# trevor-vincent/disco4est

Hardware: AMD Instinct MI355X
Metric: GDoF/s for matrix-free 3D DG stiffness apply (Ax), p=7 (higher is better)
Workload: dtype f64; 1 GPU; 3D Poisson stiffness apply on a single-tree brick, uniform level=4 (4096 elements/GPU), p=7, deg_quad=deg+0, Gauss-Legendre; general path (per-node symmetric metric streamed, affine values); dofs_per_gpu=2097152, elements_per_gpu=4096

## Files before the change

disco4est_amd/csrc/d4est_hip_direct.hip:

```cpp
#include <algorithm>
#include <type_traits>

#include "d4est_hip_direct.h"
#include "d4est_hip_internal.h"
#include "d4est_hip_tables.h"
#include "d4est_hip_wave.h"

namespace d4est_hip {

#ifndef D4EST_HIP_DIRECT_IMM_ROWS
#define D4EST_HIP_DIRECT_IMM_ROWS 1
#endif
#if D4EST_HIP_DIRECT_IMM_ROWS
#define D4EST_DIRECT_ROWS contract_rows_eo_imm
#else
#define D4EST_DIRECT_ROWS contract_rows_eo
#endif
template <int NI, int NO, bool EO, bool ANTI>
__device__ __forceinline__ void prod(const double* __restrict__ tab, const double* x, double* y) {
  if constexpr (EO) {
    constexpr int HC = (NI + 1) / 2;
    double xe[HC], xo[HC], ab[NO];
    eo_pre<NI>(x, xe, xo);
    D4EST_DIRECT_ROWS<HC, NO, false>(tab, ANTI ? xo : xe, ANTI ? xe : xo, ab);
    eo_post<NO>(ab, y);
  } else {
    contract_n<NI, NO>(tab, x, y);
  }
}

template <int NI, int NO, bool EO>
__device__ __forceinline__ void prod_pair(const double* __restrict__ tabS, const double* __restrict__ tabA, const double* x, double* yS,
                                          double* yA) {
  if constexpr (EO) {
    constexpr int HC = (NI + 1) / 2;
    double xe[HC], xo[HC], abS[NO], abA[NO];
    eo_pre<NI>(x, xe, xo);
    D4EST_DIRECT_ROWS<HC, NO, false>(tabS, xe, xo, abS);
    D4EST_DIRECT_ROWS<HC, NO, false>(tabA, xo, xe, abA);
    eo_post<NO>(abS, yS);
    eo_post<NO>(abA, yA);
  } else {
    contract_n<NI, NO>(tabS, x, yS);
    contract_n<NI, NO>(tabA, x, yA);
  }
}

template <int N>
__device__ __forceinline__ double row_dot(const double* __restrict__ drow, const double* x) {
  sdouble_ptr row = launder(drow);
  double s = row[0] * x[0];
#pragma unroll
  for (int i = 1; i < N; ++i) s = fma(row[i], x[i], s);
  return s;
}

constexpr int cmax(int a, int b) { return a > b ? a : b; }

template <int N, int NQ>
struct DirectCfg {
  static_assert(NQ >= N && NQ * NQ <= 64, "one wavefront per element: (deg_quad + 1)^2 <= 64");
  static constexpr int N2 = N * N, N3 = N2 * N, T = NQ * NQ, PN = N | 1;
  static constexpr int RS = N | 1, RQ = NQ | 1;
  static constexpr int GS = NQ * RS, YS = N * RQ;
  static constexpr int QS = T + 8, VS = N2 + 8;
  static constexpr int S_DOUBLES = cmax(cmax(cmax(8 * N * RS, 8 * GS), cmax(8 * QS, 8 * NQ * RQ)), cmax(8 * YS, 6 * VS));
  static constexpr int U_DOUBLES = PN * N2;
  static constexpr int OPSZ = N * NQ;
  static constexpr bool FULL = (N == 8 && NQ == 8);
};

constexpr int kDirectWPB = 4;

#ifndef D4EST_HIP_DIRECT_NT_MASK
#define D4EST_HIP_DIRECT_NT_MASK 7
#endif
#ifndef D4EST_HIP_DIRECT_GEOM_EARLY
#define D4EST_HIP_DIRECT_GEOM_EARLY 1
#endif
#ifndef D4EST_HIP_DIRECT_GEOM_NT_RT
#define D4EST_HIP_DIRECT_GEOM_NT_RT 1
#endif
template <int T, bool NT = false , bool HANG = false >
__device__ __forceinline__ void direct_load_geom(double* gq, int kind, bool on, int k, int sgeom, const double* __restrict__ geom,
                                                 const double* __restrict__ robin_c, bool nt_rt = false) {
#pragma unroll
  for (int c = 0; c < 7; ++c) gq[c] = 0.0;
  if (on && !(HANG && kind == 3)) {
    if (kind == 0 && robin_c) {
      gq[6] = robin_c[sgeom + k];
    } else {
      const double* __restrict__ g = geom + (size_t)7 * sgeom + k;
      if (!NT && D4EST_HIP_DIRECT_GEOM_NT_RT && nt_rt) {
        const double* gn = g;
        asm volatile("" : "+v"(gn));
#pragma unroll
        for (int c = 0; c < 7; ++c) gq[c] = __builtin_nontemporal_load(&gn[c * T]);
      } else {
#pragma unroll
        for (int c = 0; c < 7; ++c) gq[c] = ld_sel<NT>(&g[c * T]);
      }
    }
  }
}

template <int N, int NQ, bool EO, bool FUSE, int VOL = 0 >
__global__ __launch_bounds__(64 * kDirectWPB, 4) void faces_direct_kernel(const double* __restrict__ u, const double* __restrict__ ghost_qtrace,
                                                             double* __restrict__ Au, const DirectSide* __restrict__ sides,
                                                             const DirectGhostOff* __restrict__ ghost_off,
                                                             const double* __restrict__ ops, const double* __restrict__ geom,
                                                             const double* __restrict__ bndry_q, const double* __restrict__ robin_c,
                                                             const double* __restrict__ robin_r, int n_elem, int ns0, int ns_stride,
                                                             int xcd_chunk, DirectFuse cf, DirectVol vol, const int* __restrict__ elem_list) {
  using C = DirectCfg<N, NQ>;
  constexpr int N2 = C::N2, N3 = C::N3, T = C::T, PN = C::PN, RS = C::RS, RQ = C::RQ, GS = C::GS, QS = C::QS, YS = C::YS, VS = C::VS;
  constexpr bool FULL = C::FULL;
  constexpr int L0 = cmax(C::U_DOUBLES, VOL ? WaveCfg<N, NQ>::FS : 0), L1 = cmax(C::S_DOUBLES, VOL ? WaveCfg<N, NQ>::FS : 0);
  __shared__ double s_L[kDirectWPB][L0 + L1];
  const int wv = __builtin_amdgcn_readfirstlane(threadIdx.x >> 6);
  double* s_U = s_L[wv];
  double* s_S = s_L[wv] + L0;
#define tC (ops)
#define tCD (ops + C::OPSZ)
#define tE (ops + 2 * C::OPSZ)
#define tDtE (ops + 3 * C::OPSZ)
#define dr0 (ops + 4 * C::OPSZ)
  const int lane = threadIdx.x & 63;
  const int a = lane % NQ, b = lane / NQ;
  const bool on_q = FULL || lane < T, on_m = FULL || (on_q && a < N && b < N);
  const int v = blockIdx.x;
  const int slot = (xcd_chunk > 0 ? (v & 7) * xcd_chunk + (v >> 3) : v) * kDirectWPB + wv;
  if (slot >= n_elem) return;
  const int e = elem_list ? __builtin_amdgcn_readfirstlane(elem_list[slot]) : slot;
  const int ns = __builtin_amdgcn_readfirstlane(ns_stride >= 0 ? ns0 + e * ns_stride : direct_kargs()->sides[6 * (size_t)e].pad);

  {
    constexpr int UT = (N3 + 63) / 64;
    double uo[UT];
#pragma unroll
    for (int t = 0; t < UT; ++t) uo[t] = (N3 % 64 == 0 || lane + 64 * t < N3) ? u[ns + lane + 64 * t] : 0.0;
#pragma unroll
    for (int t = 0; t < UT; ++t) {
      const int idx = lane + 64 * t;
      const int i = idx % N, j = (idx / N) % N, k = idx / N2;
      if (N3 % 64 == 0 || idx < N3) s_U[i + PN * (j + N * k)] = uo[t];
    }
  }
  wave_lds_fence();
  double own_tr[6], own_nd[6];
  {
    sdouble_ptr r0 = launder(dr0), r1 = launder(dr0 + N);
#pragma unroll
    for (int d = 0; d < 3; ++d) {
      double x[N];
#pragma unroll
      for (int i = 0; i < N; ++i) {
        const int idx = (d == 0) ? i + PN * (a + N * b) : (d == 1 ? a + PN * (i + N * b) : a + PN * (b + N * i));
        x[i] = on_m ? lds_ld(&s_U[idx]) : 0.0;
      }
      own_tr[2 * d] = x[0];
      own_tr[2 * d + 1] = x[N - 1];
      double s0 = r0[0] * x[0], s1 = r1[0] * x[0];
#pragma unroll
      for (int i = 1; i < N; ++i) {
        s0 = fma(r0[i], x[i], s0);
        s1 = fma(r1[i], x[i], s1);
      }
      own_nd[2 * d] = s0;
      own_nd[2 * d + 1] = s1;
    }
  }
  wave_lds_fence();

  double facc[N];
#pragma unroll
  for (int i = 0; i < N; ++i) facc[i] = 0.0;
  int any3 = 0;

  auto dir_body = [&](auto dc) {
    constexpr int d = decltype(dc)::value;
    constexpr int t0 = (d == 0) ? 1 : 0, t1d = (d == 2) ? 1 : 2;
    typedef const DirectSide __attribute__((address_space(4))) * sside_ptr;
    const sside_ptr sd = (sside_ptr)(unsigned long long)(direct_kargs()->sides + 6 * (size_t)e);
    const int kcf[2] = {sd[2 * d].kcf, sd[2 * d + 1].kcf};
    const int sgeom[2] = {sd[2 * d].geom, sd[2 * d + 1].geom};
    if constexpr ((VOL & 16) != 0 && FUSE) any3 |= ((kcf[0] & 3) == 3) | ((kcf[1] & 3) == 3);
    double fld[8] = {own_tr[2 * d], own_tr[2 * d + 1], 0.0, 0.0, own_nd[2 * d], own_nd[2 * d + 1], 0.0, 0.0};
    double yy[2][N];
#pragma unroll
    for (int h = 0; h < 2; ++h) {
#pragma unroll
      for (int i = 0; i < N; ++i) yy[h][i] = 0.0;
      if ((kcf[h] & 3) == 1 && on_m) {
        const double* __restrict__ up = u + sd[2 * d + h].nbr_ns;
        const int dp = kcf[h] >> 6;
        const int st = (dp == 0) ? 1 : (dp == 1 ? N : N2);
        const int o0 = (dp == 0) ? N * a + N2 * b : (dp == 1 ? a + N2 * b : a + N * b);
#pragma unroll
        for (int i = 0; i < N; ++i) yy[h][i] = up[o0 + st * i];
      }
    }
#if D4EST_HIP_DIRECT_GEOM_EARLY == 2
    double gqa[2][7];
#pragma unroll
    for (int h = 0; h < 2; ++h) direct_load_geom<T, (VOL & 8) != 0 && (D4EST_HIP_DIRECT_NT_MASK & 1) != 0, (VOL & 16) != 0>(gqa[h], kcf[h] & 3, on_q, lane, sgeom[h], direct_kargs()->geom, direct_kargs()->robin_c);
#endif
#pragma unroll
    for (int h = 0; h < 2; ++h) {
      if ((kcf[h] & 3) == 1) {
        const int hi = (kcf[h] >> 5) & 1;
        fld[2 + h] = hi ? yy[h][N - 1] : yy[h][0];
        fld[6 + h] = row_dot<N>(dr0 + hi * N, yy[h]);
      }
    }
    wave_lds_fence();
    if (on_m) {
#pragma unroll
      for (int c = 0; c < 8; ++c) s_S[(c * N + b) * RS + a] = fld[c];
    }
    wave_lds_fence();
    const bool row_on = FULL || lane < 8 * N;
    const int rc = lane / N, rb = lane % N;
    double P[NQ], R[NQ];
    {
      double x[N];
#pragma unroll
      for (int i = 0; i < N; ++i) x[i] = row_on ? lds_ld(&s_S[lane * RS + i]) : 0.0;
      prod_pair<N, NQ, EO>(tC, tCD, x, P, R);
    }
// ... 55 lines not shown
        const int k = lane;
#pragma unroll
        for (int c = 0; c < 4; ++c) qm[c] = lds_ld(&s_S[c * QS + k]);
        if (kind == 1) {
          const int kp = reorder_index(code, NQ - 1, a, b);
#pragma unroll
          for (int c = 0; c < 4; ++c) qp[c] = lds_ld(&s_S[(4 + c) * QS + kp]);
        } else if (kind == 2) {
          const double* __restrict__ p = K->ghost_qtrace + K->ghost_off[6 * (size_t)e + 2 * d + h] + reorder_index(code, NQ - 1, a, b);
#pragma unroll
          for (int c = 0; c < 4; ++c) qp[c] = p[c * T];
        } else if ((VOL & 16) != 0 && kind == 3) {
        } else if (robin_c) {
          qp[0] = K->robin_r[sgeom[h] + k];
        } else {
          qp[0] = K->bndry_q[sgeom[h] + k];
        }
#if D4EST_HIP_DIRECT_GEOM_EARLY == 0
        direct_load_geom<T, (VOL & 8) != 0 && (D4EST_HIP_DIRECT_NT_MASK & 1) != 0, (VOL & 16) != 0>(gq, kind, true, k, sgeom[h], geom, robin_c);
#endif
        if constexpr ((VOL & 16) != 0) {
          const int xoff = sd[2 * d + h].nbr_ns;
          if (kind == 2 && xoff >= 0) {
            double* __restrict__ tp = const_cast<double*>((const double*)K->ghost_qtrace) + xoff;
#pragma unroll
            for (int c = 0; c < 4; ++c) tp[c * T + k] = qm[c];
          }
        }
      }
#if D4EST_HIP_DIRECT_GEOM_EARLY != 0
#pragma unroll
      for (int c = 0; c < 7; ++c) gq[c] = gqa[h][c];
#endif
      double t1 = 0.0;
#pragma unroll
      for (int i = 0; i < 3; ++i) t1 += gq[i] * qm[1 + i] + gq[3 + i] * qp[1 + i];
      const double jump = qm[0] - qp[0];
      const double w1 = (kind != 0) ? -0.5 : -1.0;
      At[h][0] = (kind == 0 && robin_c) ? gq[6] * qm[0] - qp[0] : w1 * t1 + gq[6] * jump;
#pragma unroll
      for (int l = 0; l < 3; ++l) At[h][1 + l] = w1 * gq[l] * jump;
    }
    wave_lds_fence();
    if (on_q) {
#pragma unroll
      for (int h = 0; h < 2; ++h)
#pragma unroll
        for (int c = 0; c < 4; ++c) s_S[((4 * h + c) * NQ + b) * RQ + a] = At[h][c];
    }
    wave_lds_fence();
    double Yv[N];
    {
      double row[NQ];
#pragma unroll
      for (int q = 0; q < NQ; ++q) row[q] = col_on ? lds_ld(&s_S[lane * RQ + q]) : 0.0;
      if ((cc & 3) == 1 + t0) prod<NQ, N, EO, true>(tDtE, row, Yv);
      else prod<NQ, N, EO, false>(tE, row, Yv);
    }
    wave_lds_fence();
    if (col_on) {
#pragma unroll
      for (int i = 0; i < N; ++i) s_S[cc * YS + i * RQ + aq] = Yv[i];
    }
    wave_lds_fence();
    const bool v_on = lane < 6 * N;
    const int vh = lane / (3 * N), vg = (lane / N) % 3, va = lane % N;
    double Vv[N];
    {
      double colq[NQ];
      const int f1 = (vg == 0) ? 0 : (vg == 1 ? 1 + t1d : 1 + d);
#pragma unroll
      for (int q = 0; q < NQ; ++q) {
        double t = v_on ? lds_ld(&s_S[(4 * vh + f1) * YS + va * RQ + q]) : 0.0;
        if (v_on && vg == 0) t += lds_ld(&s_S[(4 * vh + 1 + t0) * YS + va * RQ + q]);
        colq[q] = t;
      }
      if (vg == 1) prod<NQ, N, EO, true>(tDtE, colq, Vv);
      else prod<NQ, N, EO, false>(tE, colq, Vv);
    }
    wave_lds_fence();
    if (v_on) {
#pragma unroll
      for (int i = 0; i < N; ++i) s_S[(3 * vh + vg) * VS + i * N + va] = Vv[i];
    }
    wave_lds_fence();
    double acc[N];
    if (on_m) {
      const double val0 = lds_ld(&s_S[0 * VS + b * N + a]) + lds_ld(&s_S[1 * VS + b * N + a]), n0 = lds_ld(&s_S[2 * VS + b * N + a]);
      const double val1 = lds_ld(&s_S[3 * VS + b * N + a]) + lds_ld(&s_S[4 * VS + b * N + a]), n1 = lds_ld(&s_S[5 * VS + b * N + a]);
      sdouble_ptr r0 = launder(dr0), r1 = launder(dr0 + N);
#pragma unroll
      for (int i = 0; i < N; ++i) acc[i] = fma(r0[i], n0, r1[i] * n1);
      acc[0] += val0;
      acc[N - 1] += val1;
      if constexpr (d == 0) {
#pragma unroll
        for (int i = 0; i < N; ++i) s_U[i + PN * (a + N * b)] = acc[i];
      } else if constexpr (d == 1) {
#pragma unroll
        for (int i = 0; i < N; ++i) s_U[a + PN * (i + N * b)] += acc[i];
      } else if constexpr (VOL != 0) {
#pragma unroll
        for (int i = 0; i < N; ++i) facc[i] = lds_ld(&s_U[a + PN * (b + N * i)]) + acc[i];
      } else {
        DirectFuse cfl;
        if constexpr (FUSE) cfl = direct_load_fuse(direct_kargs());
        double* __restrict__ Au_ = direct_kargs()->Au;
        double av[N], rh[FUSE ? N : 1], pp[FUSE ? N : 1], uu[FUSE ? N : 1];
#pragma unroll
        for (int i = 0; i < N; ++i) {
          const size_t o = (size_t)ns + a + N * b + N2 * i;
          av[i] = Au_[o];
          if constexpr (FUSE) { rh[i] = cfl.rhs[o]; pp[i] = cfl.p[o]; uu[i] = u[o]; }
        }
#pragma unroll
        for (int i = 0; i < N; ++i) {
          const size_t o = (size_t)ns + a + N * b + N2 * i;
          const double au = av[i] + (lds_ld(&s_U[a + PN * (b + N * i)]) + acc[i]);
          Au_[o] = au;
          if constexpr (FUSE) {
            const double res = __dadd_rn(rh[i], __dmul_rn(-1.0, au));
            const double ri = __dmul_rn(cfl.alpha, res);
            const double pi = __dadd_rn(__dmul_rn(cfl.beta, pp[i]), ri);
            if (cfl.r) cfl.r[o] = ri;
            cfl.p[o] = pi;
            cfl.u_out[o] = __dadd_rn(uu[i], pi);
          }
        }
      }
    }
    wave_lds_fence();
  };
  dir_body(std::integral_constant<int, 0>{});
  dir_body(std::integral_constant<int, 1>{});
  dir_body(std::integral_constant<int, 2>{});
  if constexpr (VOL != 0) {
    static_assert(VOL == 0 || N == NQ, "fused volume term: N = NQ");
    {
      constexpr int UT = (N3 + 63) / 64;
      double uo[UT];
#pragma unroll
      for (int t = 0; t < UT; ++t) uo[t] = (N3 % 64 == 0 || lane + 64 * t < N3) ? u[ns + lane + 64 * t] : 0.0;
#pragma unroll
      for (int t = 0; t < UT; ++t) {
        const int idx = lane + 64 * t;
        const int i = idx % N, j = (idx / N) % N, k = idx / N2;
        if (N3 % 64 == 0 || idx < N3) s_U[i + PN * (j + N * k)] = uo[t];
      }
    }
    wave_lds_fence();
    {
      const DirectVol vl = direct_load_vol(direct_kargs());
      const int qs = __builtin_amdgcn_readfirstlane(vl.qs_stride >= 0 ? vl.qs0 + e * vl.qs_stride : vl.qs_list[e]);
      stiffness_wave_eo_element<N, NQ, (VOL & 3) == 2, false, (VOL & 4) != 0, (VOL & 8) != 0 && (D4EST_HIP_DIRECT_NT_MASK & 2) != 0>(s_U, s_S, vl.metric, qs, e, on_q, a, b, vl.EBf, vl.EGf, vl.EBb,
                                                                              vl.EGb, vl.affine, vl.wq, vl.cq);
    }
    if (on_m) {
      DirectFuse cfl;
      if constexpr (FUSE) cfl = direct_load_fuse(direct_kargs());
      double* __restrict__ Au_ = direct_kargs()->Au;
      const bool upd = !((VOL & 16) != 0 && any3 != 0);
      double rh[FUSE ? N : 1], pp[FUSE ? N : 1], uu[FUSE ? N : 1];
      if constexpr (FUSE) {
        if (upd) {
#pragma unroll
          for (int i = 0; i < N; ++i) {
            const size_t o = (size_t)ns + a + N * b + N2 * i;
            rh[i] = cfl.rhs[o]; pp[i] = cfl.p[o]; uu[i] = u[o];
          }
        }
      }
#pragma unroll
      for (int i = 0; i < N; ++i) {
        const size_t o = (size_t)ns + a + N * b + N2 * i;
        const double au = s_U[a + PN * (b + N * i)] + facc[i];
        if constexpr (!FUSE && (VOL & 8) != 0 && (D4EST_HIP_DIRECT_NT_MASK & 4) != 0) __builtin_nontemporal_store(au, &Au_[o]);
        else if (!FUSE || !cfl.skip_Au_store || !upd) Au_[o] = au;
        if (FUSE && upd) {
          const double res = __dadd_rn(rh[i], __dmul_rn(-1.0, au));
          const double ri = __dmul_rn(cfl.alpha, res);
          const double pi = __dadd_rn(__dmul_rn(cfl.beta, pp[i]), ri);
          if (cfl.r) cfl.r[o] = ri;
          cfl.p[o] = pi;
          cfl.u_out[o] = __dadd_rn(uu[i], pi);
        }
      }
    }
  }
#undef tC
#undef tCD
#undef tE
#undef tDtE
#undef dr0
}

static DirectHost* host_of(d4est_hip_plan* plan) { return static_cast<DirectHost*>(plan->direct); }

void direct_destroy(d4est_hip_plan* plan) {
  DirectHost* dh = host_of(plan);
  if (!dh) return;
  (void)hipFree(dh->d_sides);
  (void)hipFree(dh->d_ghost_off);
  (void)hipFree(dh->d_ops);
  (void)hipFree(dh->d_u2);
  (void)hipFree(dh->d_bnd_list); (void)hipFree(dh->d_int_list);
  delete dh;
  plan->direct = nullptr;
}

#define D4EST_HIP_DIRECT_PAIRS(X) X(2, 2) X(3, 3) X(4, 4) X(5, 5) X(6, 6) X(7, 7) X(8, 8) X(2, 3) X(3, 4) X(4, 5) X(3, 6) X(4, 6)

static bool direct_pair_built(int N, int NQ) {
#define X(N_, NQ_) if (N == N_ && NQ == NQ_) return true;
  D4EST_HIP_DIRECT_PAIRS(X)
#undef X
  return direct_mw_built(N, NQ);
}

void direct_setup(d4est_hip_plan* plan, int N, int NQ, int ns0, int ns_stride, const double* Cm, const double* CDm, const double* Em) {
  direct_destroy(plan);
  if (!direct_pair_built(N, NQ)) return;
  const int ne = plan->n_elements;
  DirectHost* dh = new DirectHost;
  dh->N = N; dh->NQ = NQ; dh->ns0 = ns0; dh->ns_stride = ns_stride;
  dh->mw = direct_mw_built(N, NQ);
  dh->eo = true;
  std::vector<double> Cv(Cm, Cm + (size_t)NQ * N), CDv(CDm, CDm + (size_t)NQ * N), Ev(Em, Em + (size_t)N * NQ);
  std::vector<double> D = Tables1D::dij(N - 1);
  std::vector<double> DtE = Tables1D::matmul(Tables1D::transpose(D, N, N), Ev, N, N, NQ);
  std::vector<double> ops;
  auto put = [&](const std::vector<double>& M, int R, int Cc, bool anti) {
    std::vector<double> t = dh->eo ? Tables1D::eo_table(M, R, Cc, anti) : Tables1D::transpose(M, R, Cc);
    t.resize((size_t)R * Cc, 0.0);
    ops.insert(ops.end(), t.begin(), t.end());
  };
  put(Cv, NQ, N, false);
  put(CDv, NQ, N, true);
  put(Ev, N, NQ, false);
  put(DtE, N, NQ, true);
  for (int i = 0; i < N; ++i) ops.push_back(D[i]);
  for (int i = 0; i < N; ++i) ops.push_back(D[(size_t)(N - 1) * N + i]);
  ops.resize(ops.size() + 16, 0.0);
  HIP_CHECK(hipMalloc(&dh->d_ops, ops.size() * sizeof(double)));
  HIP_CHECK(hipMemcpy(dh->d_ops, ops.data(), ops.size() * sizeof(double), hipMemcpyHostToDevice));
  std::vector<DirectSide> sd(6 * (size_t)ne);
  std::vector<DirectGhostOff> goff(6 * (size_t)ne, 0);
  for (int e = 0; e < ne; ++e)
    for (int f = 0; f < 6; ++f) {
      const size_t s = 6 * (size_t)e + f;
      DirectSide d{};
      const int nbr = plan->side_nbr[s];
      const int kind = (nbr == -1) ? 0 : (nbr >= 0 ? 1 : 2);
      const int fp = (kind == 0) ? 0 : plan->side_nbr_face[s];
      d.kcf = kind | ((plan->side_reorder[s] & 7) << 2) | (fp << 5);
      d.nbr_ns = (kind == 1) ? plan->nodal_stride[nbr] : 0;
      d.geom = plan->side_mortar_stride[s];
      goff[s] = (kind == 2) ? plan->ghost_trace_offset[s] : 0;
      sd[s] = d;
    }
  HIP_CHECK(hipMalloc(&dh->d_sides, std::max<size_t>(sd.size(), 1) * sizeof(DirectSide)));
  if (!sd.empty()) HIP_CHECK(hipMemcpy(dh->d_sides, sd.data(), sd.size() * sizeof(DirectSide), hipMemcpyHostToDevice));
  HIP_CHECK(hipMalloc(&dh->d_ghost_off, std::max<size_t>(goff.size(), 1) * sizeof(DirectGhostOff)));
  if (!goff.empty()) HIP_CHECK(hipMemcpy(dh->d_ghost_off, goff.data(), goff.size() * sizeof(DirectGhostOff), hipMemcpyHostToDevice));
  std::vector<int> bnd, inn;
  for (int e = 0; e < ne; ++e) {
    bool g = false;
    for (int f = 0; f < 6; ++f) g = g || plan->side_nbr[6 * (size_t)e + f] <= -2;
    (g ? bnd : inn).push_back(e);
  }
  if (!bnd.empty()) {
    dh->n_bnd = (int)bnd.size(); dh->n_int = (int)inn.size();
    HIP_CHECK(hipMalloc(&dh->d_bnd_list, bnd.size() * sizeof(int)));
    HIP_CHECK(hipMemcpy(dh->d_bnd_list, bnd.data(), bnd.size() * sizeof(int), hipMemcpyHostToDevice));
    HIP_CHECK(hipMalloc(&dh->d_int_list, std::max<size_t>(inn.size(), 1) * sizeof(int)));
    if (!inn.empty()) HIP_CHECK(hipMemcpy(dh->d_int_list, inn.data(), inn.size() * sizeof(int), hipMemcpyHostToDevice));
  }
  plan->direct = dh;
}

void direct_ghost_split(d4est_hip_plan* plan, const int** bnd_list, int* n_bnd, const int** int_list, int* n_int) {
  DirectHost* dh = host_of(plan);
  if (!dh) D4EST_HIP_ABORT("direct_ghost_split: the plan has no direct face kernel");
  *bnd_list = dh->d_bnd_list; *n_bnd = dh->n_bnd; *int_list = dh->d_int_list; *n_int = dh->n_int;
}

constexpr int kDirectMinElements = 768;

bool direct_active(const d4est_hip_plan* plan) {
  const int t = plan->tuning[D4EST_HIP_TUNE_FACE_DIRECT];
  const DirectHost* dh = static_cast<const DirectHost*>(plan->direct);
  return dh != nullptr && t != 0 && plan->tuning[D4EST_HIP_TUNE_FLUX_FAST] != 0 &&
         (t > 0 || dh->mw || plan->n_elements >= kDirectMinElements);
}

void direct_set_element_list(d4est_hip_plan* plan, const int* list_dev, int n_list) {
  DirectHost* dh = host_of(plan);
  if (!dh) D4EST_HIP_ABORT("direct_set_element_list: the plan has no direct face kernel");
  dh->d_list = list_dev;
  dh->n_list = list_dev ? n_list : 0;
}

bool direct_has_element_list(const d4est_hip_plan* plan) {
  const DirectHost* dh = static_cast<const DirectHost*>(plan->direct);
  return dh && dh->d_list != nullptr;
}

double* direct_second_vector(d4est_hip_plan* plan) {
  DirectHost* dh = host_of(plan);
  if (!dh->d_u2) HIP_CHECK(hipMalloc(&dh->d_u2, std::max<size_t>((size_t)plan->local_nodes, 1) * sizeof(double)));
  return dh->d_u2;
}

bool direct_fused_ok(const d4est_hip_plan* plan) {
  const DirectHost* dh = static_cast<const DirectHost*>(plan->direct);
  static const bool dbg = std::getenv("D4EST_HIP_DEBUG_FUSED") != nullptr;
  auto no = [&](const char* why) {
    if (dbg) std::fprintf(stderr, "[d4est_hip] whole-operator kernel not used: %s\n", why);
    return false;
  };
  if (!direct_active(plan) || !dh) return no("no direct face kernel on this plan");
  const int t = plan->tuning[D4EST_HIP_TUNE_FACE_DIRECT];
  if (!(t < 0 || t == 2)) return no("tuning key 11");
  if (dh->N != dh->NQ) return no("deg != deg_quad");
  if (!plan->has_geometry) return no("no geometry yet");
  if (plan->buckets.size() != 1) return no("more than one (deg, deg_quad) bucket");
  const Bucket& bk = plan->buckets[0];
  if (bk.N != dh->N || bk.NQ != dh->NQ || !bk.d_EBf) return no("bucket tables");
  if (bk.ns_stride >= 0 && (bk.ns0 != dh->ns0 || bk.ns_stride != dh->ns_stride)) return no("nodal offsets");
  if (bk.n_elem != plan->n_elements) return no("bucket size");
  if (dh->order_ok < 0) {
    int ok = 1;
    for (int i = 0; i < plan->n_elements && ok; ++i) ok = (plan->elem_ids[i] == i);
    dh->order_ok = ok;
  }
  if (!dh->order_ok) return no("bucket order");
  if (dh->mw) {
    if (plan->tuning[D4EST_HIP_TUNE_STIFFNESS_EO] == 0) return no("even-odd contractions switched off");
    return true;
  }
  const int tw = plan->tuning[D4EST_HIP_TUNE_STIFFNESS_WAVE];
  if (!(tw < 0 || tw == 11)) return no("tuning key 1");
  return true;
}

static void launch_direct_core(d4est_hip_plan* plan, DirectHost* dh, const Bucket& bk, bool hybrid, const int* d_qs_by_elem, const double* u,
                               const double* ghost_trace, double* Au, const DirectFuse* cf, const double* robin_c, const double* robin_r,
                               int vol_term) {
  if (!plan->has_face_geometry) D4EST_HIP_ABORT("apply flux: plan_set_mortar_geometry was not called");
  const int n = dh->d_list ? dh->n_list : plan->n_elements;
  if (n == 0) return;
  if (plan->ghost_trace_doubles > 0 && !ghost_trace) D4EST_HIP_ABORT("apply flux: plan has ghost sides but no ghost trace buffer was given");
  static const bool no_remap = std::getenv("D4EST_HIP_NO_XCD_REMAP") != nullptr;
  const int wpb = dh->mw ? 1 : kDirectWPB;
  const int n_wg = (n + wpb - 1) / wpb;
  const int chunk = (n % (8 * wpb) == 0 && !no_remap) ? n_wg / 8 : 0;
  DirectVol vol;
  int vmode = 0;
  if (vol_term) {
    if (!hybrid && !direct_fused_ok(plan)) D4EST_HIP_ABORT("direct face kernel: the fused volume term was requested on a plan that cannot take it");
    vol.metric = plan->d_metric;
    vol.EBf = bk.d_EBf; vol.EGf = bk.d_EGf; vol.EBb = bk.d_EBb; vol.EGb = bk.d_EGb;
    vol.EDq = bk.d_EDq; vol.EDqT = bk.d_EDqT;
    vol.stream = plan->stream_mode;
    {
      static const int geom_nt = [] { const char* e = std::getenv("D4EST_HIP_GEOM_NT"); return e ? std::atoi(e) : 1; }();
      if (!dh->mw && !vol.stream && (geom_nt == 2 || (geom_nt == 1 && hybrid))) vol.stream |= 2;
    }
    if (hybrid && dh->hy_qs_stride > 0) { vol.qs0 = dh->hy_qs0; vol.qs_stride = dh->hy_qs_stride; vol.qs_list = nullptr; }
    else if (hybrid) { vol.qs0 = 0; vol.qs_stride = -1; vol.qs_list = d_qs_by_elem; }
    else { vol.qs0 = bk.qs0; vol.qs_stride = bk.ns_stride >= 0 ? bk.qs_stride : -1; vol.qs_list = plan->d_qs_list + bk.elem_offset; }
    const bool aff = !hybrid && bk.affine && plan->tuning[D4EST_HIP_TUNE_AFFINE] != 0 && plan->d_metric_affine;
    if (aff) { vol.affine = plan->d_metric_affine; vol.wq = bk.d_w; }
    vmode = aff ? 2 : 1;
    if (vol_term == 2) {
      if (!plan->d_lhs_coeff) D4EST_HIP_ABORT("direct face kernel: the zeroth-order term was requested but no coefficient is set");
      vol.cq = ensure_lhs_wjc(plan);
      vmode |= 4;
    }
    const char* sm = (!aff && vol_term != 2 && (vol.stream & 1)) ? ",stream" : "";
    if (dh->mw) std::snprintf(plan->last_kernel, sizeof(plan->last_kernel), "d4est_hip::operator_mw_kernel<%d,vol%s%s> (stiffness_wave_kernel body + faces)", dh->N, aff ? ",affine" : "", sm);
    else std::snprintf(plan->last_kernel, sizeof(plan->last_kernel), "d4est_hip::faces_direct_kernel<%d,%d,vol%s%s> (faces + stiffness_wave_eo body)", dh->N, dh->NQ, aff ? ",affine" : "", sm);
  }
  if (dh->mw) {
    launch_direct_mw(plan, dh, u, ghost_trace, Au, cf, robin_c, robin_r, vmode, vol, n, chunk);
    return;
  }
  const DirectFuse cfv = cf ? *cf : DirectFuse{};
  bool done = false;
  if (vmode == 1 && (vol.stream & 1)) vmode = 9;
  if (dh->hang) {
    if (!(vmode == 1 || vmode == 9)) D4EST_HIP_ABORT("direct face kernel: the hanging-aware form exists for the plain whole operator only (vmode %d)", vmode);
    vmode |= 16;
  }
#define D4EST_HIP_DIRECT_GO(N_, NQ_, FUSE_, VOL_)                                                                             \
  hipLaunchKernelGGL((faces_direct_kernel<N_, NQ_, true, FUSE_, VOL_>), dim3(n_wg), dim3(64 * kDirectWPB), 0,     \
                     plan->stream, u, ghost_trace, Au, dh->d_sides, dh->d_ghost_off, dh->d_ops, plan->d_face_geom, plan->d_bndry,            \
                     robin_c, robin_r, n, dh->ns0, dh->ns_stride, chunk, cfv, vol, dh->d_list)
#define X(N_, NQ_)                                                                 \
  if (!done && dh->N == N_ && dh->NQ == NQ_) {                                     \
    if constexpr (N_ == NQ_) {                                                     \
      if (vmode == 1) { if (cf) D4EST_HIP_DIRECT_GO(N_, NQ_, true, 1); else D4EST_HIP_DIRECT_GO(N_, NQ_, false, 1); done = true; } \
      if (vmode == 9) { if (cf) D4EST_HIP_DIRECT_GO(N_, NQ_, true, 9); else D4EST_HIP_DIRECT_GO(N_, NQ_, false, 9); done = true; } \
      if (vmode == 17) { if (cf) D4EST_HIP_DIRECT_GO(N_, NQ_, true, 17); else D4EST_HIP_DIRECT_GO(N_, NQ_, false, 17); done = true; } \
      if (vmode == 25) { if (cf) D4EST_HIP_DIRECT_GO(N_, NQ_, true, 25); else D4EST_HIP_DIRECT_GO(N_, NQ_, false, 25); done = true; } \
      if (vmode == 2) { if (cf) D4EST_HIP_DIRECT_GO(N_, NQ_, true, 2); else D4EST_HIP_DIRECT_GO(N_, NQ_, false, 2); done = true; } \
      if (vmode == 5) { if (cf) D4EST_HIP_DIRECT_GO(N_, NQ_, true, 5); else D4EST_HIP_DIRECT_GO(N_, NQ_, false, 5); done = true; } \
      if (vmode == 6) { if (cf) D4EST_HIP_DIRECT_GO(N_, NQ_, true, 6); else D4EST_HIP_DIRECT_GO(N_, NQ_, false, 6); done = true; } \
    }                                                                              \
    if (!done) { if (cf) D4EST_HIP_DIRECT_GO(N_, NQ_, true, 0); else D4EST_HIP_DIRECT_GO(N_, NQ_, false, 0); done = true; }        \
  }
  D4EST_HIP_DIRECT_PAIRS(X)
#undef X
#undef D4EST_HIP_DIRECT_GO
  if (!done) D4EST_HIP_ABORT("direct face kernel: no instance for N = %d, NQ = %d", dh->N, dh->NQ);
  static bool occ_done = false;
  if (!occ_done && std::getenv("D4EST_HIP_DEBUG_OCC")) {
    occ_done = true;
    int nb = -1, nv = -1;
    hipFuncAttributes at{}, av{};
    (void)hipOccupancyMaxActiveBlocksPerMultiprocessor(&nb, reinterpret_cast<const void*>(faces_direct_kernel<8, 8, true, false, 0>), 64 * kDirectWPB, 0);
    (void)hipFuncGetAttributes(&at, reinterpret_cast<const void*>(faces_direct_kernel<8, 8, true, false, 0>));
    (void)hipOccupancyMaxActiveBlocksPerMultiprocessor(&nv, reinterpret_cast<const void*>(faces_direct_kernel<8, 8, true, false, 1>), 64 * kDirectWPB, 0);
    (void)hipFuncGetAttributes(&av, reinterpret_cast<const void*>(faces_direct_kernel<8, 8, true, false, 1>));
    std::fprintf(stderr, "[d4est_hip] occupancy: faces_direct<8,8> %d workgroups of %d waves per CU (regs %d, lds %zu, scratch %zu); with the volume term %d (regs %d, lds %zu, scratch %zu)\n",
                 nb, kDirectWPB, at.numRegs, at.sharedSizeBytes, at.localSizeBytes, nv, av.numRegs, av.sharedSizeBytes, av.localSizeBytes);
  }
  HIP_CHECK(hipGetLastError());
}

void launch_direct_faces(d4est_hip_plan* plan, const double* u, const double* ghost_trace, double* Au, const DirectFuse* cf,
                         const double* robin_c, const double* robin_r, int vol_term) {
  DirectHost* dh = host_of(plan);
  if (!dh) D4EST_HIP_ABORT("direct face kernel: the plan has no direct tables");
  launch_direct_core(plan, dh, plan->buckets[0], false, nullptr, u, ghost_trace, Au, cf, robin_c, robin_r, vol_term);
}

struct HybridHost {
  std::vector<DirectHost*> dh;
  std::vector<int*> d_clean;
  std::vector<int> n_clean;
  DirectSide* d_sides = nullptr;
  DirectGhostOff* d_ghost_off = nullptr;
  int* d_qs_by_elem = nullptr;
  int *d_dirty = nullptr, *d_ring = nullptr;
  int n_dirty = 0, n_ring = 0, n_clean_total = 0;
  std::vector<int> h_dirty, h_ring;
  int *d_ns_dirty = nullptr, *d_qs_dirty = nullptr;
  std::vector<int> dirty_off, dirty_cnt;
  char path[96] = "";
  double* d_u2 = nullptr;
  bool hang = false;
  std::vector<hipStream_t> side;
  std::vector<hipEvent_t> done;
  hipEvent_t fork = nullptr;
};
static HybridHost* hybrid_of(const d4est_hip_plan* plan) { return static_cast<HybridHost*>(plan->hybrid); }

void hybrid_destroy(d4est_hip_plan* plan) {
  HybridHost* hh = hybrid_of(plan);
  if (!hh) return;
  for (DirectHost* d : hh->dh)
    if (d) { (void)hipFree(d->d_ops); delete d; }
  for (int* p : hh->d_clean) (void)hipFree(p);
  for (hipStream_t st : hh->side) (void)hipStreamDestroy(st);
  for (hipEvent_t ev : hh->done) (void)hipEventDestroy(ev);
  if (hh->fork) (void)hipEventDestroy(hh->fork);
  (void)hipFree(hh->d_sides); (void)hipFree(hh->d_ghost_off); (void)hipFree(hh->d_qs_by_elem); (void)hipFree(hh->d_dirty); (void)hipFree(hh->d_ring);
  (void)hipFree(hh->d_ns_dirty); (void)hipFree(hh->d_qs_dirty); (void)hipFree(hh->d_u2);
  delete hh;
  plan->hybrid = nullptr;
}

bool hybrid_pair_built(int N, int NQ) { return N == NQ && direct_pair_built(N, NQ); }

template <typename T>
static T* hy_upload(const std::vector<T>& v) {
  T* d = nullptr;
  HIP_CHECK(hipMalloc(&d, std::max<size_t>(v.size(), 1) * sizeof(T)));
  if (!v.empty()) HIP_CHECK(hipMemcpy(d, v.data(), v.size() * sizeof(T), hipMemcpyHostToDevice));
  return d;
}

void hybrid_setup(d4est_hip_plan* plan, const std::vector<char>& clean, const std::vector<const double*>& C, const std::vector<const double*>& CD,
                  const std::vector<const double*>& E, const std::vector<HybridSideOverride>* ov, const char* form) {
  hybrid_destroy(plan);
  const int ne = plan->n_elements;
  HybridHost* hh = new HybridHost;
  const size_t nb = plan->buckets.size();
  hh->dh.assign(nb, nullptr); hh->d_clean.assign(nb, nullptr); hh->n_clean.assign(nb, 0);
  hh->dirty_off.assign(nb, 0); hh->dirty_cnt.assign(nb, 0);
  std::vector<DirectSide> sd(6 * (size_t)ne);
  std::vector<DirectGhostOff> goff(6 * (size_t)ne, 0);
  for (int e = 0; e < ne; ++e)
    for (int f = 0; f < 6; ++f) {
      const size_t s = 6 * (size_t)e + f;
      DirectSide d{};
      const int nbr = plan->side_nbr[s];
      const int kind = (nbr == -1) ? 0 : (nbr >= 0 ? 1 : 2);
      const int fp = (kind == 0) ? 0 : plan->side_nbr_face[s];
      d.kcf = kind | ((plan->side_reorder[s] & 7) << 2) | (fp << 5);
      d.nbr_ns = (kind == 1) ? plan->nodal_stride[nbr] : 0;
      d.geom = plan->side_mortar_stride[s];
      d.pad = (f == 0) ? plan->nodal_stride[e] : 0;
      if (ov && clean[e] && (*ov)[s].kind >= 0) {
        const HybridSideOverride& o = (*ov)[s];
        d.kcf = o.kind | ((plan->side_reorder[s] & 7) << 2);
        if (o.kind == 2) { d.nbr_ns = o.export_off; d.geom = o.geom; goff[s] = o.goff; }
        hh->hang = true;
      }
      sd[s] = d;
    }
  hh->d_sides = hy_upload(sd);
  hh->d_ghost_off = hy_upload(goff);
  hh->d_qs_by_elem = hy_upload(plan->quad_stride);
  std::vector<int> dirty, ns_dirty, qs_dirty;
  for (size_t b = 0; b < nb; ++b) {
    const Bucket& bk = plan->buckets[b];
    std::vector<int> cl;
    hh->dirty_off[b] = (int)ns_dirty.size();
    for (int i = 0; i < bk.n_elem; ++i) {
      const int e = plan->elem_ids[bk.elem_offset + i];
      if (clean[e]) cl.push_back(e);
      else { ns_dirty.push_back(plan->nodal_stride[e]); qs_dirty.push_back(plan->quad_stride[e]); }
    }
    hh->dirty_cnt[b] = (int)ns_dirty.size() - hh->dirty_off[b];
    if (cl.empty()) continue;
    std::sort(cl.begin(), cl.end());
    DirectHost* dh = new DirectHost;
    const int N = bk.N, NQ = bk.NQ;
    dh->N = N; dh->NQ = NQ; dh->ns0 = 0; dh->ns_stride = -1;
    dh->mw = direct_mw_built(N, NQ);
    dh->eo = true;
    dh->hang = hh->hang;
    std::vector<double> Cv(C[b], C[b] + (size_t)NQ * N), CDv(CD[b], CD[b] + (size_t)NQ * N), Ev(E[b], E[b] + (size_t)N * NQ);
// ... 159 lines not shown
```

disco4est_amd/csrc/d4est_hip_internal.h:

```cpp
#pragma once
#include <hip/hip_runtime.h>

#include <cstdio>
#include <cstdlib>
#include <vector>

#include "../../include/d4est_hip.h"

#define D4EST_HIP_ABORT(...)                                   \
  do {                                                         \
    std::fprintf(stderr, "[D4EST_HIP_ABORT] ");                \
    std::fprintf(stderr, __VA_ARGS__);                         \
    std::fprintf(stderr, " (%s:%d)\n", __FILE__, __LINE__);    \
    std::abort();                                              \
  } while (0)

#define HIP_CHECK(expr)                                                              \
  do {                                                                               \
    hipError_t _e = (expr);                                                          \
    if (_e != hipSuccess) D4EST_HIP_ABORT("%s failed: %s", #expr, hipGetErrorString(_e)); \
  } while (0)

namespace d4est_hip {

struct Bucket {
  int deg = 0, deg_quad = 0;
  int N = 0, NQ = 0;
  int n_elem = 0;
  int elem_offset = 0;
  double* d_B = nullptr;
  double* d_G = nullptr;
  double* d_D = nullptr;
  double* d_w = nullptr;
  double* d_BT = nullptr;
  double* d_GT = nullptr;
  double* d_DT = nullptr;
  int ns0 = 0, ns_stride = -1, qs0 = 0, qs_stride = -1;
  bool affine = false;
  double* d_EBf = nullptr;
  double* d_EGf = nullptr;
  double* d_EBb = nullptr;
  double* d_EGb = nullptr;
  double* d_EDq = nullptr;
  double* d_EDqT = nullptr;
  double* d_M = nullptr;
  double* d_MT = nullptr;
  double* d_Minv = nullptr;
  double* d_MinvT = nullptr;
  double* d_Binv = nullptr;
  double* d_BinvT = nullptr;
  double* d_wGL = nullptr;
};

}

struct d4est_hip_plan {
  int n_elements = 0;
  int local_nodes = 0;
  int local_nodes_quad = 0;
  int quad_type = 0;
  hipStream_t stream = nullptr;
  int n_cus = 0;
  char last_kernel[128] = "";

  std::vector<int> deg, deg_quad, nodal_stride, quad_stride;
  std::vector<d4est_hip::Bucket> buckets;

  std::vector<int> elem_ids;
  int* d_elem_ids = nullptr;
  int* d_ns_list = nullptr;
  int* d_qs_list = nullptr;

  bool has_geometry = false;
  double* d_J = nullptr;
  int* d_face_stride = nullptr;
  int face_nodes = 0;
  double* d_metric = nullptr;
  double* d_metric_affine = nullptr;
  int* d_nonaffine = nullptr;

  bool has_faces = false, has_face_geometry = false;
  int n_ghost = 0;
  std::vector<int> ghost_deg, ghost_deg_quad;
  std::vector<int> side_nbr, side_nbr_face, side_reorder, side_mortar_stride, side_bndry_stride;
  std::vector<int> side_hang, side_sub, side_nbr4, side_orientation;
  int total_mortar_nodes = 0, total_bndry_nodes = 0;
  long long local_trace_doubles = 0, ghost_trace_doubles = 0;
  int* d_side_desc = nullptr;
  void* d_elem_desc = nullptr;
  std::vector<long long> rec_qoff, rec_goff;
  std::vector<int> rec_len, side_first_rec;
  std::vector<long long> trace_offset, ghost_trace_offset;
  double* d_face_ops = nullptr;
  double* d_face_geom = nullptr;
  double* d_bndry = nullptr;
  double* d_trace = nullptr;
  double sipg_prefactor = 10.0;
  int sipg_penalty_fcn = 0;
  int max_face_lds_doubles = 0;
  bool face_fast = false;
  void* direct = nullptr;
  void* hybrid = nullptr;

  double *d_work_p = nullptr, *d_work_d = nullptr, *d_work_r = nullptr, *d_reduce = nullptr, *d_ghost_trace = nullptr;
  const double* d_lhs_coeff = nullptr;
  double* d_lhs_c = nullptr;
  double* d_lhs_wjc = nullptr;
  bool lhs_wjc_valid = false;
  double* d_work_m = nullptr;
  const double* d_lhs_blocks = nullptr;
  long long* d_lhs_block_off = nullptr;
  void* lhs_chain = nullptr;
  hipStream_t side_stream = nullptr;
  hipEvent_t ev_fork = nullptr, ev_join = nullptr;
  hipGraphExec_t cheby_graph = nullptr;
  struct { const void *u, *rhs, *Au, *r; int iter, flag; double lmin, lmax; hipStream_t stream; } cheby_graph_key = {};
  d4est_hip_exchange_fn exchange_fn = nullptr;
  d4est_hip_allreduce_fn allreduce_fn = nullptr;
  void* comm_ctx = nullptr;

  unsigned long long op_generation = 0;
  bool quad_aliased = false;
  int stream_mode = 0;
  bool bc_inhomogeneous = false;

  int tuning[D4EST_HIP_TUNE_COUNT] = {-1, -1, -1, -1, -1, -1, -1, -1, -1, -1, -1, -1, -1, -1, -1, -1};

  void* krylov = nullptr;

  double* d_scratch = nullptr;
  size_t scratch_doubles = 0;

  bool est_requested = false;
  int est_fcn[3] = {-1, -1, -1};
  double est_prefactor = 0.0;
  void* est = nullptr;

  double* h_stage = nullptr;
  double* d_host[4] = {nullptr, nullptr, nullptr, nullptr};
};

namespace d4est_hip {
struct TreeMapParams;
struct CellDesc;
void launch_analytic_geometry(d4est_hip_plan* plan, const TreeMapParams& P, const CellDesc* d_cells, double root_len);
void faces_set_geometry_analytic(d4est_hip_plan* plan, const TreeMapParams& P, const std::vector<CellDesc>& elem,
                                 const std::vector<CellDesc>& ghost, double root_len);

void launch_metric_precombine(d4est_hip_plan* plan, const double* d_J, const double* d_rst);
void launch_stiffness(d4est_hip_plan* plan, const double* u, double* Au);
void launch_stiffness_view(d4est_hip_plan* plan, const double* u, double* Au, int* ns_list_view, int* qs_list_view, const int* view_offset,
                           const int* view_count);
void launch_mass_like(d4est_hip_plan* plan, int mode, const double* in, double* out, const double* coeff = nullptr, int which = 0);
void launch_brick_geometry(d4est_hip_plan* plan, const int* d_elem_dq, double root_len, const double* extents);
void launch_numerical_geometry(d4est_hip_plan* plan, const double* d_xyz);
void faces_set_geometry_brick(d4est_hip_plan* plan, const int* d_elem_dq, double root_len, const double* extents);
void launch_slicer_lift(d4est_hip_plan* plan, const double* in, double* out, int face, int lift);
void launch_dij(d4est_hip_plan* plan, const double* in, double* out, int dir, int transpose);
void launch_dudr(d4est_hip_plan* plan, const double* u, double* d0, double* d1, double* d2);

void faces_setup(d4est_hip_plan* plan);
void faces_set_geometry(d4est_hip_plan* plan, const double* sj, const double* n, const double* drst_m, const double* drst_p,
                        const double* hm, const double* hp, int on_device);
int reorient_face_order(int f_m, int f_p, int o, int i);
int face_reorder_code(int f_m, int f_p, int o);
void faces_set_dirichlet(d4est_hip_plan* plan, const double* g_lobatto, int on_device);
void faces_set_robin(d4est_hip_plan* plan, const double* coeff_quad, const double* rhs_quad, int on_device);
void launch_traces(d4est_hip_plan* plan, const double* u, double* trace, bool ghost, const int* elist = nullptr, int n_list = 0, int parts = 3 );
struct ChebyFuse {
  const double* rhs = nullptr;
  double* p = nullptr;
  double* u = nullptr;
  double* u_out = nullptr;
  int skip_Au_store = 0;
  double* r = nullptr;
  double alpha = 0.0, beta = 0.0;
};
bool flux_can_fuse_update(d4est_hip_plan* plan);

struct DirectFuse {
  const double* rhs = nullptr;
  double* p = nullptr;
  double* u_out = nullptr;
  double* r = nullptr;
  double alpha = 0.0, beta = 0.0;
  int skip_Au_store = 0;
  int pad = 0;
};
void direct_setup(d4est_hip_plan* plan, int N, int NQ, int ns0, int ns_stride, const double* C, const double* CD, const double* E);
void direct_destroy(d4est_hip_plan* plan);
bool direct_active(const d4est_hip_plan* plan);
double* direct_second_vector(d4est_hip_plan* plan);
void direct_set_element_list(d4est_hip_plan* plan, const int* list_dev, int n_list);
bool direct_has_element_list(const d4est_hip_plan* plan);
bool direct_fused_ok(const d4est_hip_plan* plan);
void direct_ghost_split(d4est_hip_plan* plan, const int** bnd_list, int* n_bnd, const int** int_list, int* n_int);
void launch_direct_faces(d4est_hip_plan* plan, const double* u, const double* ghost_trace, double* Au, const DirectFuse* cf,
                         const double* robin_c, const double* robin_r, int vol_term);
void launch_flux_direct(d4est_hip_plan* plan, const double* u, const double* ghost_trace, double* Au, const DirectFuse* cf = nullptr,
                        int vol_term = 0);
void launch_flux(d4est_hip_plan* plan, const double* trace, const double* ghost_trace, double* Au, const ChebyFuse* cf = nullptr,
                 const int* elist = nullptr, int n_list = 0, int parts = 3);
bool hybrid_pair_built(int N, int NQ);
struct HybridSideOverride { int kind; long long goff; int export_off; int geom; };
void hybrid_setup(d4est_hip_plan* plan, const std::vector<char>& clean, const std::vector<const double*>& C, const std::vector<const double*>& CD,
                  const std::vector<const double*>& E, const std::vector<HybridSideOverride>* ov = nullptr, const char* form = "hanging-aware");
bool hybrid_hanging(const d4est_hip_plan* plan);
void hybrid_host_lists(const d4est_hip_plan* plan, const std::vector<int>** dirty, const std::vector<int>** ring);
void hybrid_destroy(d4est_hip_plan* plan);
bool hybrid_active(const d4est_hip_plan* plan);
const char* hybrid_path(const d4est_hip_plan* plan);
void hybrid_lists(const d4est_hip_plan* plan, const int** dirty, int* n_dirty, const int** ring, int* n_ring);
void launch_hybrid_clean(d4est_hip_plan* plan, const double* u, const double* ghost_trace, double* Au, const double* robin_c, const double* robin_r,
                         int phase, const DirectFuse* cf = nullptr);
bool hybrid_can_fuse_update(const d4est_hip_plan* plan);
double* hybrid_second_vector(d4est_hip_plan* plan);
void launch_flux_units(d4est_hip_plan* plan, const double* trace, const double* ghost_trace, double* Au, const ChebyFuse* cf);
bool faces_have_units(d4est_hip_plan* plan);
bool faces_hp(d4est_hip_plan* plan);
bool faces_hp_split(d4est_hip_plan* plan);
void launch_hybrid_dirty_stiffness(d4est_hip_plan* plan, const double* u, double* Au);
void launch_flux_hybrid_clean(d4est_hip_plan* plan, const double* u, const double* ghost_trace, double* Au, int phase, const DirectFuse* cf = nullptr);
void faces_destroy(d4est_hip_plan* plan);
struct EstMortar {
  int elem;
  int kind;
  int code;
  int NQ;
  int gidx;
  int S, off, off_p, Ttot;
  int deg_m, deg_p;
  int N;
  int offC, ops_hp;
  int bstride;
  int u_shift;
  double fm, fp;
  long long qoff, nbr_qoff;
};
void faces_estimator_mortars(d4est_hip_plan* plan, std::vector<EstMortar>& out, std::vector<int>& elem_first, const double** face_ops,
                             const double** hp_ops);
void launch_traces_all(d4est_hip_plan* plan, const double* u, double* trace);
void launch_boundary_gather(d4est_hip_plan* plan, const double* vol, double* out);
void estimator_setup(d4est_hip_plan* plan, const double* sj, const double* n, const double* drst_m, const double* drst_p, const double* hm,
                     const double* hp);
void estimator_destroy(d4est_hip_plan* plan);
void estimator_compute(d4est_hip_plan* plan, const double* u, const double* ghost_trace, const double* residual, const double* diam,
                       const double* g_lobatto, double* eta2, double* terms);

void apply_operator(d4est_hip_plan* plan, const double* u, double* Au, const ChebyFuse* cf = nullptr, bool lhs_term = true);
void launch_residual(d4est_hip_plan* plan, int n, const double* rhs, const double* Au, double* r);
void launch_residual_inplace(d4est_hip_plan* plan, int n, const double* rhs, double* r);
void launch_residual_inplace_sub(d4est_hip_plan* plan, int n, const double* a, double* r);
void ensure_solver_workspace(d4est_hip_plan* plan);
void add_lhs_mass_term(d4est_hip_plan* plan, const double* u, double* Au);
void add_lhs_blocks_term(d4est_hip_plan* plan, const double* u, double* Au);
void add_lhs_chain_term(d4est_hip_plan* plan, const double* u, double* Au);
void lhs_chain_destroy(d4est_hip_plan* plan);
inline bool lhs_extra_term(const d4est_hip_plan* plan) { return plan->d_lhs_blocks != nullptr || plan->lhs_chain != nullptr; }
const double* ensure_lhs_wjc(d4est_hip_plan* plan);
void launch_copy_blocks(hipStream_t stream, int n_blocks, const double* src, const long long* src_off, double* dst,
                        const long long* dst_off, const int* len);
void launch_dot(d4est_hip_plan* plan, int n, const double* x, const double* y, double* out_dev);
void launch_cheby_update(d4est_hip_plan* plan, int n, const double* rhs, const double* Au, double alpha, double beta, double* r,
                         double* p, double* u);
void cheby_iterate(d4est_hip_plan* plan, double* u, const double* rhs, double* Au, double* r, int iter, double lmin, double lmax,
                   int compute_residual_at_end);
double cg_eigs(d4est_hip_plan* plan, double* u, const double* rhs, double* Au, int imax, int use_new, double* hist_out);

int cg_solve(d4est_hip_plan* plan, double* u, const double* rhs, double* Au, int imax, double atol, double rtol, double* hist_out);
int fcg_solve(d4est_hip_plan* plan, double* u, const double* rhs, double* Au, int imax, double atol, double rtol, d4est_hip_pc_fn pc,
              void* pc_ctx, double* hist_out);
void krylov_destroy(d4est_hip_plan* plan);


}
```

disco4est_amd/csrc/d4est_hip_volume.hip:

```cpp
#include <algorithm>
#include <mutex>
#include <unordered_map>
#include <cstring>

#include "d4est_hip_internal.h"
#include "d4est_hip_maps.h"
#include "d4est_hip_tables.h"
#include "d4est_hip_wave.h"
#include "d4est_hip_mwave.h"

namespace d4est_hip {

template <int N, int NQ>
struct VolCfg {
  static_assert(NQ >= N, "quadrature degree below polynomial degree is served by the generic path");
  static constexpr int PL = NQ * NQ;
  static constexpr int EPB = (PL <= 64) ? (64 / PL) : 1;
  static constexpr int THREADS = (PL <= 64) ? 64 : ((PL + 63) / 64) * 64;
  static constexpr int PN = N | 1;
  static constexpr int PQ = NQ | 1;
  static constexpr int FS = NQ * NQ * PQ;
  static constexpr int LDS_PER_ELEM = 3 * FS;
  static constexpr size_t LDS_BYTES = (size_t)EPB * LDS_PER_ELEM * sizeof(double);
};
// ... 301 lines not shown
      for (int j = 0; j < N; ++j) x[j] = lds_ld(&R1[j + PN * (a + NQ * b)]);
      contract_n_part<N, NQ, HQ>(BopT, q0, x, t_bb);
      contract_n_part<N, NQ, HQ>(GopT, q0, x, t_gb);
#pragma unroll
      for (int j = 0; j < N; ++j) x[j] = lds_ld(&R2[j + PN * (a + NQ * b)]);
      contract_n_part<N, NQ, HQ>(BopT, q0, x, t_bg);
    }
    __syncthreads();
    if (on2) {
#pragma unroll
      for (int jq = 0; jq < HQ; ++jq) {
        R0[b + PN * (a + NQ * (q0 + jq))] = t_bg[jq];
        R1[b + PN * (a + NQ * (q0 + jq))] = t_gb[jq];
        R2[b + PN * (a + NQ * (q0 + jq))] = t_bb[jq];
      }
    }
  }
  __syncthreads();

  double fr[HQ], fs[HQ], ft[HQ];
  if (active) {
    double x[N];
#pragma unroll
    for (int k = 0; k < N; ++k) x[k] = lds_ld(&R0[k + PN * (a + NQ * b)]);
    contract_n_part<N, NQ, HQ>(BopT, q0, x, fr);
#pragma unroll
    for (int k = 0; k < N; ++k) x[k] = lds_ld(&R1[k + PN * (a + NQ * b)]);
    contract_n_part<N, NQ, HQ>(BopT, q0, x, fs);
#pragma unroll
    for (int k = 0; k < N; ++k) x[k] = lds_ld(&R2[k + PN * (a + NQ * b)]);
    contract_n_part<N, NQ, HQ>(GopT, q0, x, ft);
#pragma unroll
    for (int kq = 0; kq < HQ; ++kq) {
      const double r = fr[kq], s = fs[kq], t = ft[kq];
      fr[kq] = mreg[0][kq] * r + mreg[1][kq] * s + mreg[2][kq] * t;
      fs[kq] = mreg[1][kq] * r + mreg[3][kq] * s + mreg[4][kq] * t;
      ft[kq] = mreg[2][kq] * r + mreg[4][kq] * s + mreg[5][kq] * t;
    }
  }
  __syncthreads();
  if (active) {
#pragma unroll
    for (int kq = 0; kq < HQ; ++kq) {
      R0[q0 + kq + PQ * (a + NQ * b)] = fr[kq];
      R1[q0 + kq + PQ * (a + NQ * b)] = fs[kq];
      R2[q0 + kq + PQ * (a + NQ * b)] = ft[kq];
    }
  }
  __syncthreads();
  {
    double x[NQ], ca[HN], cb[HN], cc[HN];
    if (active) {
#pragma unroll
      for (int kq = 0; kq < NQ; ++kq) x[kq] = lds_ld(&R0[kq + PQ * (a + NQ * b)]);
      contract_t_part<NQ, N, HN, false>(Bop, n0, x, ca);
#pragma unroll
      for (int kq = 0; kq < NQ; ++kq) x[kq] = lds_ld(&R1[kq + PQ * (a + NQ * b)]);
      contract_t_part<NQ, N, HN, false>(Bop, n0, x, cb);
#pragma unroll
      for (int kq = 0; kq < NQ; ++kq) x[kq] = lds_ld(&R2[kq + PQ * (a + NQ * b)]);
      contract_t_part<NQ, N, HN, false>(Gop, n0, x, cc);
    }
    __syncthreads();
    if (active) {
#pragma unroll
      for (int k = 0; k < HN; ++k) {
        R0[b + PQ * (a + NQ * (n0 + k))] = ca[k];
        R1[b + PQ * (a + NQ * (n0 + k))] = cb[k];
        R2[b + PQ * (a + NQ * (n0 + k))] = cc[k];
      }
    }
  }
  __syncthreads();
  {
    double x[NQ], ar[HN], bs[HN];
    const bool on6 = active && b < N;
    if (on6) {
#pragma unroll
      for (int jq = 0; jq < NQ; ++jq) x[jq] = lds_ld(&R0[jq + PQ * (a + NQ * b)]);
      contract_t_part<NQ, N, HN, false>(Bop, n0, x, ar);
#pragma unroll
      for (int jq = 0; jq < NQ; ++jq) x[jq] = lds_ld(&R1[jq + PQ * (a + NQ * b)]);
      contract_t_part<NQ, N, HN, false>(Gop, n0, x, bs);
#pragma unroll
      for (int jq = 0; jq < NQ; ++jq) x[jq] = lds_ld(&R2[jq + PQ * (a + NQ * b)]);
      contract_t_part<NQ, N, HN, true>(Bop, n0, x, bs);
    }
    __syncthreads();
    if (on6) {
#pragma unroll
      for (int j = 0; j < HN; ++j) {
        R0[a + PQ * (n0 + j + N * b)] = ar[j];
        R1[a + PQ * (n0 + j + N * b)] = bs[j];
      }
    }
  }
  __syncthreads();
  if (active && a < N && b < N) {
    double x[NQ], o[HN];
#pragma unroll
    for (int iq = 0; iq < NQ; ++iq) x[iq] = lds_ld(&R0[iq + PQ * (a + N * b)]);
    contract_t_part<NQ, N, HN, false>(Gop, n0, x, o);
#pragma unroll
    for (int iq = 0; iq < NQ; ++iq) x[iq] = lds_ld(&R1[iq + PQ * (a + N * b)]);
    contract_t_part<NQ, N, HN, true>(Bop, n0, x, o);
#pragma unroll
    for (int i = 0; i < HN; ++i) R2[n0 + i + PN * (a + N * b)] = o[i];
  }
  __syncthreads();
  if (active) {
#pragma unroll
    for (int idx = te + h * PL; idx < N3; idx += 2 * PL) {
      const int i = idx % N, j = (idx / N) % N, k = idx / (N * N);
      Au[ns + idx] = lds_ld(&R2[i + PN * (j + N * k)]);
    }
  }
}


template <int N, int NQ>
__global__ __launch_bounds__(64, 4) void stiffness_wave2_kernel(
    const double* __restrict__ u, double* __restrict__ Au, const double* __restrict__ metric,
    const int* __restrict__ ns_list, const int* __restrict__ qs_list, int n_bucket, const double* __restrict__ Bop,
    const double* __restrict__ Gop, const double* __restrict__ BopT, const double* __restrict__ GopT, int stagger) {
  if (stagger > 0 && ((blockIdx.x >> 8) & 1)) {
    for (int s_ = 0; s_ < stagger; ++s_) __builtin_amdgcn_s_sleep(16);
  }
  using C = WaveCfg<N, NQ>;
  constexpr int PL = C::PL, PN = C::PN, PQ = C::PQ, FS = C::FS;
  constexpr int N3 = N * N * N, NQ3 = NQ * NQ * NQ;
  extern __shared__ __attribute__((aligned(16))) double smem[];

  const int tid = threadIdx.x;
  const int slot = tid / PL;
  const int te = tid - slot * PL;
  const int a = te % NQ, b = te / NQ;
  const int ei = blockIdx.x * C::EPB + slot;
  const bool active = (slot < C::EPB) && (ei < n_bucket);
  double* R0 = smem + (active ? slot : 0) * C::LDS_PER_ELEM;
  double* R1 = R0 + FS;
  int ns = 0, qs = 0;
  if (active) {
    ns = ns_list[ei];
    qs = qs_list[ei];
    load_element_image<N, PL, PN>(R0, u + ns, te);
  }
  __syncthreads();
  stiffness_wave2_element<N, NQ, true>(R0, R1, metric, qs, active, a, b, Bop, Gop, BopT, GopT);
  if (active) {
    store_element_image<N, PL, PN>(Au + ns, R0, te);
  }
}

template <int N, int NQ, bool AFF = false>
__global__ __launch_bounds__(64, 4) void stiffness_wave_eo_kernel(
    const double* __restrict__ u, double* __restrict__ Au, const double* __restrict__ metric,
    const int* __restrict__ ns_list, const int* __restrict__ qs_list, int n_bucket, const double* __restrict__ EBf,
    const double* __restrict__ EGf, const double* __restrict__ EBb, const double* __restrict__ EGb, int ns0, int ns_stride,
    int qs0, int qs_stride, const double* __restrict__ affine = nullptr, const double* __restrict__ wq = nullptr) {
  using C = WaveCfg<N, NQ>;
  constexpr int PL = C::PL, PN = C::PN, PQ = C::PQ, FS = C::FS;
  constexpr int N3 = N * N * N, NQ3 = NQ * NQ * NQ;
  constexpr int HN = N / 2, HQ = NQ / 2;
  extern __shared__ __attribute__((aligned(16))) double smem[];

  const int tid = threadIdx.x;
  const int slot = tid / PL;
  const int te = tid - slot * PL;
  const int a = te % NQ, b = te / NQ;
  const int ei = blockIdx.x * C::EPB + slot;
  const bool active = (slot < C::EPB) && (ei < n_bucket);
  double* R0 = smem + (active ? slot : 0) * C::LDS_PER_ELEM;
  double* R1 = R0 + FS;
  int ns = 0, qs = 0;
  if (active) {
    if (ns_stride >= 0) {
      ns = ns0 + ei * ns_stride;
      qs = qs0 + ei * qs_stride;
    } else {
      ns = ns_list[ei];
      qs = qs_list[ei];
    }
    if (C::EPB == 1) {
      ns = __builtin_amdgcn_readfirstlane(ns);
      qs = __builtin_amdgcn_readfirstlane(qs);
    }
    load_element_image<N, PL, PN>(R0, u + ns, te);
  }
  __syncthreads();
  stiffness_wave_eo_element<N, NQ, AFF, true>(R0, R1, metric, qs, ei, active, a, b, EBf, EGf, EBb, EGb, affine, wq);
  if (active) {
    store_element_image<N, PL, PN>(Au + ns, R0, te);
  }
}

struct WaveEoMulti {
  static constexpr int MAXB = 7;
  int n = 0;
  int wg_end[MAXB] = {};
  int N[MAXB] = {};
  int n_elem[MAXB] = {};
  int elem_offset[MAXB] = {};
  const double* EBf[MAXB] = {};
  const double* EGf[MAXB] = {};
  const double* EBb[MAXB] = {};
  const double* EGb[MAXB] = {};
  const double* wq[MAXB] = {};
};

template <int N, bool AFF>
__device__ __forceinline__ void wave_eo_multi_body(double* smem, int wg, const double* __restrict__ u, double* __restrict__ Au,
                                                   const double* __restrict__ metric, const int* __restrict__ ns_list,
                                                   const int* __restrict__ qs_list, int n_bucket, const double* __restrict__ EBf,
                                                   const double* __restrict__ EGf, const double* __restrict__ EBb,
                                                   const double* __restrict__ EGb, const double* __restrict__ affine,
                                                   const double* __restrict__ wq) {
  using C = WaveCfg<N, N>;
  constexpr int PL = C::PL, PN = C::PN, FS = C::FS;
  const int tid = threadIdx.x;
  const int slot = tid / PL;
  const int te = tid - slot * PL;
  const int a = te % N, b = te / N;
  const int ei = wg * C::EPB + slot;
  const bool active = (slot < C::EPB) && (ei < n_bucket);
  double* R0 = smem + (active ? slot : 0) * C::LDS_PER_ELEM;
  double* R1 = R0 + FS;
  int ns = 0, qs = 0;
  if (active) {
    ns = ns_list[ei];
    qs = qs_list[ei];
    if (C::EPB == 1) {
      ns = __builtin_amdgcn_readfirstlane(ns);
      qs = __builtin_amdgcn_readfirstlane(qs);
    }
    load_element_image<N, PL, PN>(R0, u + ns, te);
  }
  __syncthreads();
  stiffness_wave_eo_element<N, N, AFF, true>(R0, R1, metric, qs, ei, active, a, b, EBf, EGf, EBb, EGb, affine, wq);
  if (active) {
    store_element_image<N, PL, PN>(Au + ns, R0, te);
  }
}

template <bool AFF>
__global__ __launch_bounds__(64, 4) void stiffness_wave_eo_multi_kernel(const double* __restrict__ u, double* __restrict__ Au,
                                                                        const double* __restrict__ metric,
                                                                        const int* __restrict__ ns_list_all,
                                                                        const int* __restrict__ qs_list_all,
                                                                        const double* __restrict__ affine_all, WaveEoMulti A) {
  extern __shared__ __attribute__((aligned(16))) double smem[];
  const int blk = blockIdx.x;
  int bi = 0;
  while (bi + 1 < A.n && blk >= A.wg_end[bi]) ++bi;
  const int wg = blk - (bi > 0 ? A.wg_end[bi - 1] : 0);
  const int off = A.elem_offset[bi], nb = A.n_elem[bi];
  const double* EBf = A.EBf[bi];
  const double* EGf = A.EGf[bi];
  const double* EBb = A.EBb[bi];
  const double* EGb = A.EGb[bi];
  const double* wq = A.wq[bi];
  const double* aff = AFF ? affine_all + (size_t)6 * off : nullptr;
#define D4EST_CASE(N_)                                                                                                            \
  case N_:                                                                                                                        \
    wave_eo_multi_body<N_, AFF>(smem, wg, u, Au, metric, ns_list_all + off, qs_list_all + off, nb, EBf, EGf, EBb, EGb, aff, wq);   \
    break;
  switch (A.N[bi]) {
    D4EST_CASE(2) D4EST_CASE(3) D4EST_CASE(4) D4EST_CASE(5) D4EST_CASE(6) D4EST_CASE(7) D4EST_CASE(8)
    default: break;
  }
#undef D4EST_CASE
}

template <int N, bool NT>
__device__ __forceinline__ void mw_multi_body(double* smem, int ei, const double* __restrict__ u, double* __restrict__ Au,
                                              const double* __restrict__ metric, const int* __restrict__ ns_list, const int* __restrict__ qs_list,
                                              int n_bucket, const double* __restrict__ EBb, const double* __restrict__ EBf,
                                              const double* __restrict__ EDq, const double* __restrict__ EDqT) {
  using C = WaveCfg<N, N>;
  constexpr int PL = C::PL, PN = C::PN;
  const int te = threadIdx.x;
  const int a = te % N, b = te / N;
  const bool active = (te < PL) && (ei < n_bucket);
  double* R0 = smem;
  double* R1 = R0 + C::FS;
  int ns = 0, qs = 0;
  if (ei < n_bucket) {
    ns = __builtin_amdgcn_readfirstlane(ns_list[ei]);
    qs = __builtin_amdgcn_readfirstlane(qs_list[ei]);
  }
  if (active) load_element_image<N, PL, PN>(R0, u + ns, te);
  stiffness_mw_element_cg<N, false, false, NT>(R0, R1, metric, qs, ei, active, te, a, b, EBb, EBf, EDq, EDqT, nullptr, nullptr);
  if (active) store_element_image<N, PL, PN, NT>(Au + ns, R0, te);
}

template <int THREADS, bool NT>
__global__ __launch_bounds__(THREADS, D4EST_HIP_MW_WAVES) void stiffness_mw_multi_kernel(const double* __restrict__ u, double* __restrict__ Au,
                                                                                        const double* __restrict__ metric,
                                                                                        const int* __restrict__ ns_list_all,
                                                                                        const int* __restrict__ qs_list_all, WaveEoMulti A) {
  extern __shared__ __attribute__((aligned(16))) double smem[];
  const int blk = blockIdx.x;
  int bi = 0;
  while (bi + 1 < A.n && blk >= A.wg_end[bi]) ++bi;
  const int ei = blk - (bi > 0 ? A.wg_end[bi - 1] : 0);
  const int off = A.elem_offset[bi], nb = A.n_elem[bi];
  const double* EBf = A.EBf[bi];
  const double* EDqT = A.EGf[bi];
  const double* EBb = A.EBb[bi];
  const double* EDq = A.EGb[bi];
#define D4EST_CASE(N_)                                                                                                  \
  case N_:                                                                                                              \
    if constexpr (WaveCfg<N_, N_>::THREADS == THREADS)                                                                  \
      mw_multi_body<N_, NT>(smem, ei, u, Au, metric, ns_list_all + off, qs_list_all + off, nb, EBb, EBf, EDq, EDqT);    \
    break;
  switch (A.N[bi]) {
    D4EST_CASE(9) D4EST_CASE(10) D4EST_CASE(11) D4EST_CASE(12) D4EST_CASE(13)
    default: break;
  }
#undef D4EST_CASE
}


template <bool NT>
__global__ __launch_bounds__(128, D4EST_HIP_MW_WAVES) void stiffness_all_multi_kernel(const double* __restrict__ u, double* __restrict__ Au,
                                                                                    const double* __restrict__ metric,
                                                                                    const int* __restrict__ ns_list_all,
                                                                                    const int* __restrict__ qs_list_all, WaveEoMulti A) {
  extern __shared__ __attribute__((aligned(16))) double smem[];
  const int blk = blockIdx.x;
  int bi = 0;
  while (bi + 1 < A.n && blk >= A.wg_end[bi]) ++bi;
  const int wgb = blk - (bi > 0 ? A.wg_end[bi - 1] : 0);
  const int off = A.elem_offset[bi], nb = A.n_elem[bi];
  const double* EBf = A.EBf[bi];
  const double* EGf = A.EGf[bi];
  const double* EBb = A.EBb[bi];
  const double* EGb = A.EGb[bi];
  const int wv = __builtin_amdgcn_readfirstlane(threadIdx.x >> 6);
#define D4EST_CASE_EO(N_)                                                                                                              \
  case N_: {                                                                                                                           \
    using C = WaveCfg<N_, N_>;                                                                                                         \
    constexpr int PL = C::PL, PN = C::PN, FS = C::FS;                                                                                  \
    const int tid = threadIdx.x & 63, slot = tid / PL, te = tid - slot * PL;                                                           \
    const int ei = (2 * wgb + wv) * C::EPB + slot;                                                                                     \
    const bool active = (slot < C::EPB) && (ei < nb);                                                                                  \
    double* R0 = smem + wv * (C::EPB * C::LDS_PER_ELEM) + (active ? slot : 0) * C::LDS_PER_ELEM;                                       \
    double* R1 = R0 + FS;                                                                                                              \
    int ns = 0, qs = 0;                                                                                                                \
    if (active) {                                                                                                                      \
      ns = ns_list_all[off + ei];                                                                                                      \
      qs = qs_list_all[off + ei];                                                                                                      \
      if (C::EPB == 1) { ns = __builtin_amdgcn_readfirstlane(ns); qs = __builtin_amdgcn_readfirstlane(qs); }                           \
      load_element_image<N_, PL, PN>(R0, u + ns, te);                                                                                  \
    }                                                                                                                                  \
    wave_lds_fence();                                                                                                                  \
    stiffness_wave_eo_element<N_, N_, false, false>(R0, R1, metric, qs, ei, active, te % N_, te / N_, EBf, EGf, EBb, EGb, nullptr, nullptr); \
    if (active) store_element_image<N_, PL, PN>(Au + ns, R0, te);                                                                      \
  } break;
#define D4EST_CASE_MW(N_)                                                                                                              \
  case N_:                                                                                                                             \
    mw_multi_body<N_, NT>(smem, wgb, u, Au, metric, ns_list_all + off, qs_list_all + off, nb, EBb, EBf, EGb, EGf);                     \
    break;
  switch (A.N[bi]) {
    D4EST_CASE_EO(2) D4EST_CASE_EO(3) D4EST_CASE_EO(4) D4EST_CASE_EO(5) D4EST_CASE_EO(6) D4EST_CASE_EO(7) D4EST_CASE_EO(8)
    D4EST_CASE_MW(9) D4EST_CASE_MW(10) D4EST_CASE_MW(11)
    default: break;
  }
#undef D4EST_CASE_EO
#undef D4EST_CASE_MW
}

typedef double mfma_d4v __attribute__((ext_vector_type(4)));
#define D4_MFMA(a_, b_, c_) __builtin_amdgcn_mfma_f64_16x16x4f64((a_), (b_), (c_), 0, 0, 0)

struct Mfma16Cfg {
  static constexpr int JS = 17, KS = 16 * 17, FS = 16 * KS;
  static constexpr size_t LDS_BYTES = (size_t)3 * FS * sizeof(double);
};

template <int N, bool AFF = false>
__global__ __launch_bounds__(512, 1) void stiffness_mfma16_kernel(const double* __restrict__ u, double* __restrict__ Au,
                                                                   const double* __restrict__ metric, const int* __restrict__ ns_list,
                                                                   const int* __restrict__ qs_list, int n_bucket,
                                                                   const double* __restrict__ Bop, const double* __restrict__ Gop,
                                                                   const double* __restrict__ affine = nullptr,
                                                                   const double* __restrict__ wq = nullptr, int stream = 0) {
  constexpr int JS = Mfma16Cfg::JS, KS = Mfma16Cfg::KS, FS = Mfma16Cfg::FS;
  extern __shared__ __attribute__((aligned(16))) double smem[];
  const int tid = threadIdx.x, wave = tid >> 6, lane = tid & 63, q = lane >> 4, c = lane & 15;
  double Bn[4], Gn[4], Bt[4], Gt[4];
#pragma unroll
  for (int s = 0; s < 4; ++s) {
    const bool in = (c < N) && (4 * s + q < N);
    Bn[s] = in ? Bop[c * N + 4 * s + q] : 0.0;
    Gn[s] = in ? Gop[c * N + 4 * s + q] : 0.0;
    Bt[s] = in ? Bop[(4 * s + q) * N + c] : 0.0;
    Gt[s] = in ? Gop[(4 * s + q) * N + c] : 0.0;
  }
  const mfma_d4v zero = {0.0, 0.0, 0.0, 0.0};
  double xa[2][4];
  int e = blockIdx.x;
  if (e < n_bucket) {
    const double* ue = u + ns_list[e];
#pragma unroll
    for (int h = 0; h < 2; ++h)
#pragma unroll
      for (int s = 0; s < 4; ++s)
        xa[h][s] = (c < N && 4 * s + q < N && 2 * wave + h < N) ? ue[(4 * s + q) + N * c + N * N * (2 * wave + h)] : 0.0;
  }
  for (; e < n_bucket; e += gridDim.x) {
    const int ns = ns_list[e];
    const double* me = metric + (size_t)6 * (AFF ? 0 : qs_list[e]);
    double mt[6][4];
    auto tile_metric = [&](int ct, double (*dst)[4]) {
      if constexpr (AFF) {
        const double* __restrict__ cc = affine + (size_t)6 * e;
        const double wcj = (c < N && ct < N) ? wq[c] * wq[ct] : 0.0;
#pragma unroll
        for (int v = 0; v < 4; ++v) {
          const double w3 = (4 * v + q < N) ? wcj * wq[4 * v + q] : 0.0;
#pragma unroll
          for (int m = 0; m < 6; ++m) dst[m][v] = w3 * cc[m];
        }
      } else {
        with_ld(stream != 0, [&](auto ld) {
#pragma unroll
          for (int m = 0; m < 6; ++m)
#pragma unroll
            for (int v = 0; v < 4; ++v)
              dst[m][v] = (c < N && ct < N && 4 * v + q < N) ? ld(&me[m * (N * N * N) + c + N * ct + N * N * (4 * v + q)]) : 0.0;
        });
      }
    };
    tile_metric(2 * wave, mt);
#pragma unroll
    for (int h = 0; h < 2; ++h) {
      const int k = 2 * wave + h;
      if (k >= N) continue;
      mfma_d4v pb = zero, pg = zero;
#pragma unroll
      for (int s = 0; s < 4; ++s) {
        pb = D4_MFMA(xa[h][s], Bn[s], pb);
        pg = D4_MFMA(xa[h][s], Gn[s], pg);
      }
      mfma_d4v za = zero, zb = zero, zc = zero;
#pragma unroll
      for (int s = 0; s < 4; ++s) {
        za = D4_MFMA(Bn[s], pb[s], za);
        zb = D4_MFMA(Bn[s], pg[s], zb);
        zc = D4_MFMA(Gn[s], pb[s], zc);
      }
      double* z = smem + k * KS + c;
#pragma unroll
      for (int v = 0; v < 4; ++v) {
        z[JS * (4 * v + q)] = zb[v];
        z[FS + JS * (4 * v + q)] = zc[v];
        z[2 * FS + JS * (4 * v + q)] = za[v];
      }
    }
    {
      const int e_next = e + (int)gridDim.x;
      if (e_next < n_bucket) {
        const double* un = u + ns_list[e_next];
#pragma unroll
        for (int h = 0; h < 2; ++h)
#pragma unroll
          for (int s = 0; s < 4; ++s)
            xa[h][s] = (c < N && 4 * s + q < N && 2 * wave + h < N) ? un[(4 * s + q) + N * c + N * N * (2 * wave + h)] : 0.0;
      }
    }
    __syncthreads();
    double mt2[6][4];
    tile_metric(2 * wave + 1, mt2);
#pragma unroll
    for (int h = 0; h < 2; ++h) {
      const int ct = 2 * wave + h;
      if (ct >= N) continue;
      const double* z = smem + JS * ct + c;
      mfma_d4v tr = zero, ts = zero, tt = zero;
#pragma unroll
      for (int s = 0; s < 4; ++s) {
        const int off = (4 * s + q) * KS;
        tr = D4_MFMA(Bn[s], z[off], tr);
        ts = D4_MFMA(Bn[s], z[FS + off], ts);
        tt = D4_MFMA(Gn[s], z[2 * FS + off], tt);
      }
      mfma_d4v fr, fs, ft;
#pragma unroll
      for (int v = 0; v < 4; ++v) {
        fr[v] = mt[0][v] * tr[v] + mt[1][v] * ts[v] + mt[2][v] * tt[v];
        fs[v] = mt[1][v] * tr[v] + mt[3][v] * ts[v] + mt[4][v] * tt[v];
        ft[v] = mt[2][v] * tr[v] + mt[4][v] * ts[v] + mt[5][v] * tt[v];
      }
      if (h == 0) {
#pragma unroll
        for (int m = 0; m < 6; ++m)
#pragma unroll
          for (int v = 0; v < 4; ++v) mt[m][v] = mt2[m][v];
      }
      mfma_d4v wr = zero, ws = zero, wt = zero;
#pragma unroll
      for (int s = 0; s < 4; ++s) {
        wr = D4_MFMA(Bt[s], fr[s], wr);
        ws = D4_MFMA(Bt[s], fs[s], ws);
        wt = D4_MFMA(Gt[s], ft[s], wt);
      }
      double* w = smem + JS * ct + c;
#pragma unroll
      for (int v = 0; v < 4; ++v) {
// ... 303 lines not shown
  const int ei = blockIdx.x * C::EPB + slot;
  const bool active = (slot < C::EPB) && (ei < n_bucket);
  double* R0 = smem + (active ? slot : 0) * C::LDS_PER_ELEM;
  double* R1 = R0 + C::FS;
  int ns = 0;
  if (active) ns = ns_list[ei];
  if (active) {
    load_element_image<N, PL, PN>(R0, u + ns, te);
  }
  __syncthreads();
  if (active) {
    double x[N], y[N];
#pragma unroll
    for (int k = 0; k < N; ++k) x[k] = lds_ld(&R0[a + PN * (b + N * k)]);
    contract_n<N, N>(DopT, x, y);
#pragma unroll
    for (int k = 0; k < N; ++k) d2[ns + a + N * (b + N * k)] = y[k];
#pragma unroll
    for (int j = 0; j < N; ++j) x[j] = lds_ld(&R0[a + PN * (j + N * b)]);
    contract_n<N, N>(DopT, x, y);
#pragma unroll
    for (int j = 0; j < N; ++j) d1[ns + a + N * (j + N * b)] = y[j];
#pragma unroll
    for (int i = 0; i < N; ++i) x[i] = lds_ld(&R0[i + PN * (a + N * b)]);
    contract_n<N, N>(DopT, x, y);
#pragma unroll
    for (int i = 0; i < N; ++i) R1[i + PN * (a + N * b)] = y[i];
  }
  __syncthreads();
  if (active) {
    store_element_image<N, PL, PN>(d0 + ns, R1, te);
  }
}

__global__ __launch_bounds__(256) void generic_dudr_kernel(const double* __restrict__ u, double* __restrict__ d0,
                                                           double* __restrict__ d1, double* __restrict__ d2,
                                                           const int* __restrict__ ns_list, int n_bucket, int N,
                                                           const double* __restrict__ Dop) {
  for (int ei = blockIdx.x; ei < n_bucket; ei += gridDim.x) {
    const int ns = ns_list[ei];
    GenDims dn = {{N, N, N}};
    gen_apply(Dop, N, N, 1, 0, u + ns, dn, d0 + ns, false);
    gen_apply(Dop, N, N, 1, 1, u + ns, dn, d1 + ns, false);
    gen_apply(Dop, N, N, 1, 2, u + ns, dn, d2 + ns, false);
  }
}

__global__ __launch_bounds__(256) void generic_dij_kernel(const double* __restrict__ in, double* __restrict__ out,
                                                          const int* __restrict__ ns_list, int n_bucket, int N,
                                                          const double* __restrict__ Dop, int dir, int transpose) {
  for (int ei = blockIdx.x; ei < n_bucket; ei += gridDim.x) {
    const int ns = ns_list[ei];
    GenDims dn = {{N, N, N}};
    gen_apply(Dop, N, transpose ? 1 : N, transpose ? N : 1, dir, in + ns, dn, out + ns, false);
  }
}

__global__ __launch_bounds__(256) void metric_precombine_kernel(const double* __restrict__ J, const double* __restrict__ rst,
                                                                size_t local_nodes_quad, const int* __restrict__ qs_list,
                                                                int n_bucket, int NQ,
                                                                const double* __restrict__ wq, double* __restrict__ metric,
                                                                double* __restrict__ affine ,
                                                                int* __restrict__ nonaffine_flag) {
  const int NQ3 = NQ * NQ * NQ;
  __shared__ double g0[6];
  for (int ei = blockIdx.x; ei < n_bucket; ei += gridDim.x) {
    const int qs = qs_list[ei];
    double* m = metric + (size_t)6 * qs;
    if (threadIdx.x < 6) {
      int i = 0, j = 0, c = 0;
      for (int a = 0; a < 3; ++a)
        for (int b = a; b < 3; ++b) {
          if (c == (int)threadIdx.x) { i = a; j = b; }
          ++c;
        }
      double sum = 0.0;
      for (int d = 0; d < 3; ++d)
        sum += rst[(size_t)(3 * i + d) * local_nodes_quad + qs] * rst[(size_t)(3 * j + d) * local_nodes_quad + qs];
      g0[threadIdx.x] = J[qs] * sum;
      affine[(size_t)6 * ei + threadIdx.x] = g0[threadIdx.x];
    }
    __syncthreads();
    double scale = 0.0;
    for (int c = 0; c < 6; ++c) scale = fmax(scale, fabs(g0[c]));
    bool deviates = false;
    for (int q = threadIdx.x; q < NQ3; q += blockDim.x) {
      const int iq = q % NQ, jq = (q / NQ) % NQ, kq = q / (NQ * NQ);
      const double Jq = J[qs + q];
      const double wj = (wq[kq] * (wq[jq] * wq[iq])) * Jq;
      double r[3][3];
#pragma unroll
      for (int i = 0; i < 3; ++i)
#pragma unroll
        for (int j = 0; j < 3; ++j) r[i][j] = rst[(size_t)(3 * i + j) * local_nodes_quad + qs + q];
      int c = 0;
#pragma unroll
      for (int i = 0; i < 3; ++i)
#pragma unroll
        for (int j = i; j < 3; ++j) {
          const double gsum = r[i][0] * r[j][0] + r[i][1] * r[j][1] + r[i][2] * r[j][2];
          m[(size_t)c * NQ3 + q] = wj * gsum;
          if (fabs(Jq * gsum - g0[c]) > 1e-15 * scale) deviates = true;
          ++c;
        }
    }
    if (deviates) atomicOr(nonaffine_flag, 1);
    __syncthreads();
  }
}

#define D4EST_HIP_FAST_PAIRS(X) \
  X(2, 2) X(3, 3) X(4, 4) X(5, 5) X(6, 6) X(7, 7) X(8, 8) X(9, 9) X(10, 10) X(11, 11) X(12, 12) \
  X(13, 13) X(14, 14) X(15, 15) X(16, 16)                                                       \
  X(2, 3) X(3, 4) X(4, 5) X(8, 9) X(3, 6) X(4, 6) X(8, 10)

#define D4EST_HIP_BIG_PAIRS(X) X(17, 17) X(18, 18) X(19, 19) X(20, 20)

template <typename K>
static void set_lds_limit(K kernel, size_t bytes) {
  if (bytes <= 64 * 1024) return;
  static std::mutex mu;
  static std::unordered_map<const void*, size_t> done;
  const void* key = reinterpret_cast<const void*>(kernel);
  std::lock_guard<std::mutex> lock(mu);
  auto it = done.find(key);
  if (it != done.end() && it->second >= bytes) return;
  HIP_CHECK(hipFuncSetAttribute(key, hipFuncAttributeMaxDynamicSharedMemorySize, (int)bytes));
  done[key] = bytes;
}

static void ensure_scratch(d4est_hip_plan* plan, size_t doubles) {
  if (plan->scratch_doubles >= doubles) return;
  if (plan->d_scratch) HIP_CHECK(hipFree(plan->d_scratch));
  HIP_CHECK(hipMalloc(&plan->d_scratch, doubles * sizeof(double)));
  plan->scratch_doubles = doubles;
}

static void launch_generic(d4est_hip_plan* plan, const Bucket& bk, int mode, const double* in, double* out,
                           const double* coeff = nullptr, const double* op = nullptr, const int* qs_list = nullptr, int NQe = -1,
                           const double* wts = nullptr) {
  if (!wts) wts = bk.d_w;
  if (!op) op = bk.d_B;
  if (!qs_list) qs_list = plan->d_qs_list + bk.elem_offset;
  if (NQe < 0) NQe = bk.NQ;
  const int NM = bk.N > NQe ? bk.N : NQe;
  const size_t per_block = (size_t)8 * NM * NM * NM;
  const int grid = bk.n_elem < 1024 ? bk.n_elem : 1024;
  ensure_scratch(plan, per_block * grid);
  hipLaunchKernelGGL(generic_volume_kernel, dim3(grid), dim3(256), 0, plan->stream, mode, in, out, plan->d_metric, plan->d_J,
                     plan->d_ns_list + bk.elem_offset, qs_list, bk.n_elem, bk.N, NQe, op, bk.d_G, wts, plan->d_scratch,
                     per_block, coeff);
}

template <int N, int NQ>
static void launch_stiffness_wave(d4est_hip_plan* plan, const Bucket& bk, bool use_pf, const double* u, double* Au) {
  if constexpr (NQ * NQ <= 64 && NQ >= N) {
    using W = WaveCfg<N, NQ>;
    const int grid = (bk.n_elem + W::EPB - 1) / W::EPB;
    const int ts = plan->tuning[D4EST_HIP_TUNE_STIFFNESS_STAGGER];
    const int cus_ = plan->n_cus > 0 ? plan->n_cus : 256;
    (void)cus_;
    const int stagger = ts < 0 ? 0 : ts;
    const int tw_ = plan->tuning[D4EST_HIP_TUNE_STIFFNESS_WAVE];
    const bool use_affine = bk.affine && plan->tuning[D4EST_HIP_TUNE_AFFINE] != 0 && bk.d_EBf && (tw_ == 11 || tw_ < 0);
    if (use_affine) {
      std::snprintf(plan->last_kernel, sizeof(plan->last_kernel), "d4est_hip::stiffness_wave_eo_kernel<%d,%d,affine>", N, NQ);
      hipLaunchKernelGGL((stiffness_wave_eo_kernel<N, NQ, true>), dim3(grid), dim3(64), W::LDS_BYTES, plan->stream, u, Au, plan->d_metric,
                           plan->d_ns_list + bk.elem_offset, plan->d_qs_list + bk.elem_offset, bk.n_elem, bk.d_EBf, bk.d_EGf,
                           bk.d_EBb, bk.d_EGb, bk.ns0, bk.ns_stride, bk.qs0, bk.qs_stride,
                           plan->d_metric_affine + (size_t)6 * bk.elem_offset, bk.d_w);
    } else if ((tw_ == 11 || tw_ < 0) && bk.d_EBf) {
      std::snprintf(plan->last_kernel, sizeof(plan->last_kernel), "d4est_hip::stiffness_wave_eo_kernel<%d,%d>", N, NQ);
      hipLaunchKernelGGL((stiffness_wave_eo_kernel<N, NQ>), dim3(grid), dim3(64), W::LDS_BYTES, plan->stream, u, Au, plan->d_metric,
                           plan->d_ns_list + bk.elem_offset, plan->d_qs_list + bk.elem_offset, bk.n_elem, bk.d_EBf, bk.d_EGf,
                           bk.d_EBb, bk.d_EGb, bk.ns0, bk.ns_stride, bk.qs0, bk.qs_stride);
    } else if (tw_ == 3 || tw_ < 0) {
      std::snprintf(plan->last_kernel, sizeof(plan->last_kernel), "d4est_hip::stiffness_wave2_kernel<%d,%d>", N, NQ);
      hipLaunchKernelGGL((stiffness_wave2_kernel<N, NQ>), dim3(grid), dim3(64), W::LDS_BYTES, plan->stream, u, Au, plan->d_metric,
                         plan->d_ns_list + bk.elem_offset, plan->d_qs_list + bk.elem_offset, bk.n_elem, bk.d_B, bk.d_G, bk.d_BT,
                         bk.d_GT, stagger);
    } else if (plan->tuning[D4EST_HIP_TUNE_STIFFNESS_WAVE] == 2 && N % 2 == 0 && NQ % 2 == 0) {
      std::snprintf(plan->last_kernel, sizeof(plan->last_kernel), "d4est_hip::stiffness_pair_kernel<%d,%d>", N, NQ);
      if constexpr (N % 2 == 0 && NQ % 2 == 0)
        hipLaunchKernelGGL((stiffness_pair_kernel<N, NQ>), dim3(grid), dim3(128), (W::LDS_BYTES / 2) * 3, plan->stream, u, Au,
                           plan->d_metric, plan->d_ns_list + bk.elem_offset, plan->d_qs_list + bk.elem_offset, bk.n_elem,
                           bk.d_B, bk.d_G, bk.d_BT, bk.d_GT);
    } else if (use_pf) {
      std::snprintf(plan->last_kernel, sizeof(plan->last_kernel), "d4est_hip::stiffness_wave_kernel<%d,%d,true>", N, NQ);
      hipLaunchKernelGGL((stiffness_wave_kernel<N, NQ, true>), dim3(grid), dim3(64), W::LDS_BYTES, plan->stream, u, Au,
                         plan->d_metric, plan->d_ns_list + bk.elem_offset, plan->d_qs_list + bk.elem_offset, bk.n_elem,
                         bk.d_B, bk.d_G, bk.d_BT, bk.d_GT, stagger);
    } else {
      std::snprintf(plan->last_kernel, sizeof(plan->last_kernel), "d4est_hip::stiffness_wave_kernel<%d,%d,false>", N, NQ);
      hipLaunchKernelGGL((stiffness_wave_kernel<N, NQ, false>), dim3(grid), dim3(64), W::LDS_BYTES, plan->stream, u, Au,
                         plan->d_metric, plan->d_ns_list + bk.elem_offset, plan->d_qs_list + bk.elem_offset, bk.n_elem,
                         bk.d_B, bk.d_G, bk.d_BT, bk.d_GT, stagger);
    }
  }
}

static void launch_stiffness_mfma16(d4est_hip_plan* plan, const Bucket& bk, const double* u, double* Au) {
  const bool aff = bk.affine && plan->tuning[D4EST_HIP_TUNE_AFFINE] != 0 && plan->d_metric_affine && bk.N == 16;
  std::snprintf(plan->last_kernel, sizeof(plan->last_kernel), "d4est_hip::stiffness_mfma16_kernel<%d%s> (512 threads, v_mfma_f64_16x16x4)", bk.N,
                aff ? ",affine" : "");
  const int cus = plan->n_cus > 0 ? plan->n_cus : 256;
  const int grid = bk.n_elem < cus ? bk.n_elem : cus;
  auto go = [&](auto kern) {
    set_lds_limit(kern, Mfma16Cfg::LDS_BYTES);
    hipLaunchKernelGGL(kern, dim3(grid), dim3(512), Mfma16Cfg::LDS_BYTES, plan->stream, u, Au, plan->d_metric,
                       plan->d_ns_list + bk.elem_offset, plan->d_qs_list + bk.elem_offset, bk.n_elem, bk.d_B, bk.d_G,
                       aff ? plan->d_metric_affine + (size_t)6 * bk.elem_offset : (const double*)nullptr, bk.d_w, plan->stream_mode);
  };
  if (aff) go(stiffness_mfma16_kernel<16, true>);
  else if (bk.N == 16) go(stiffness_mfma16_kernel<16>);
  else if (bk.N == 15) go(stiffness_mfma16_kernel<15>);
  else if (bk.N == 14) go(stiffness_mfma16_kernel<14>);
  else go(stiffness_mfma16_kernel<13>);
}

static unsigned launch_stiffness_multi(d4est_hip_plan* plan, const double* u, double* Au) {
  const int tw = plan->tuning[D4EST_HIP_TUNE_STIFFNESS_WAVE];
  if (!(tw < 0 || tw == 11) || plan->tuning[D4EST_HIP_TUNE_STIFFNESS_PREFETCH] > 0) return 0u;
  unsigned covered = 0u;
  for (int aff = 0; aff < 2; ++aff) {
    WaveEoMulti A;
    size_t lds = 0;
    unsigned mine = 0u;
    int wgs = 0;
    for (size_t i = 0; i < plan->buckets.size() && i < 32; ++i) {
      const Bucket& bk = plan->buckets[i];
      if (bk.n_elem == 0 || bk.N != bk.NQ || bk.N < 2 || bk.N > 8 || !bk.d_EBf || A.n == WaveEoMulti::MAXB) continue;
      const bool use_affine = bk.affine && plan->tuning[D4EST_HIP_TUNE_AFFINE] != 0 && plan->d_metric_affine;
      if ((int)use_affine != aff || !(bk.n_elem <= 8192 || use_affine)) continue;
      size_t l = 0;
      int epb = 1;
#define X(N_) if (bk.N == N_) { l = WaveCfg<N_, N_>::LDS_BYTES; epb = WaveCfg<N_, N_>::EPB; }
      X(2) X(3) X(4) X(5) X(6) X(7) X(8)
#undef X
      lds = std::max(lds, l);
      wgs += (bk.n_elem + epb - 1) / epb;
      const int j = A.n++;
      A.wg_end[j] = wgs; A.N[j] = bk.N; A.n_elem[j] = bk.n_elem; A.elem_offset[j] = bk.elem_offset;
      A.EBf[j] = bk.d_EBf; A.EGf[j] = bk.d_EGf; A.EBb[j] = bk.d_EBb; A.EGb[j] = bk.d_EGb; A.wq[j] = bk.d_w;
      mine |= 1u << i;
    }
    if (A.n < 2) continue;
    std::snprintf(plan->last_kernel, sizeof(plan->last_kernel), "d4est_hip::stiffness_wave_eo_multi_kernel<%s> (%d buckets)", aff ? "affine" : "general", A.n);
    if (aff)
      hipLaunchKernelGGL((stiffness_wave_eo_multi_kernel<true>), dim3(wgs), dim3(64), lds, plan->stream, u, Au, plan->d_metric, plan->d_ns_list,
                         plan->d_qs_list, plan->d_metric_affine, A);
    else
      hipLaunchKernelGGL((stiffness_wave_eo_multi_kernel<false>), dim3(wgs), dim3(64), lds, plan->stream, u, Au, plan->d_metric, plan->d_ns_list,
                         plan->d_qs_list, (const double*)nullptr, A);
    covered |= mine;
  }
  return covered;
}

static unsigned launch_stiffness_multi_mw(d4est_hip_plan* plan, const double* u, double* Au) {
  if (plan->tuning[D4EST_HIP_TUNE_STIFFNESS_BIGP] >= 0 && plan->tuning[D4EST_HIP_TUNE_STIFFNESS_BIGP] != 1) return 0u;
  if (plan->tuning[D4EST_HIP_TUNE_STIFFNESS_EO] == 0) return 0u;
  unsigned covered = 0u;
  for (int threads = 128; threads <= 192; threads += 64) {
    WaveEoMulti A;
    size_t lds = 0;
    unsigned mine = 0u;
    int wgs = 0;
    for (size_t i = 0; i < plan->buckets.size() && i < 32; ++i) {
      const Bucket& bk = plan->buckets[i];
      if (bk.n_elem == 0 || bk.N != bk.NQ || bk.N < 9 || bk.N > 13 || !bk.d_EDq || A.n == WaveEoMulti::MAXB) continue;
      if (bk.affine && plan->tuning[D4EST_HIP_TUNE_AFFINE] != 0 && plan->d_metric_affine) continue;
      const int th = ((bk.N * bk.N + 63) / 64) * 64;
      if (th != threads) continue;
      lds = std::max(lds, (size_t)2 * bk.N * bk.N * (bk.N | 1) * sizeof(double));
      wgs += bk.n_elem;
      const int j = A.n++;
      A.wg_end[j] = wgs; A.N[j] = bk.N; A.n_elem[j] = bk.n_elem; A.elem_offset[j] = bk.elem_offset;
      A.EBf[j] = bk.d_EBf; A.EGf[j] = bk.d_EDqT; A.EBb[j] = bk.d_EBb; A.EGb[j] = bk.d_EDq; A.wq[j] = bk.d_w;
      mine |= 1u << i;
    }
    if (A.n < 2) continue;
    std::snprintf(plan->last_kernel, sizeof(plan->last_kernel), "d4est_hip::stiffness_mw_multi_kernel<%d> (%d buckets)", threads, A.n);
    auto go = [&](auto kern) {
      set_lds_limit(kern, lds);
      hipLaunchKernelGGL(kern, dim3(wgs), dim3(threads), lds, plan->stream, u, Au, plan->d_metric, plan->d_ns_list, plan->d_qs_list, A);
    };
    if (threads == 128) { if (plan->stream_mode) go(stiffness_mw_multi_kernel<128, true>); else go(stiffness_mw_multi_kernel<128, false>); }
    else { if (plan->stream_mode) go(stiffness_mw_multi_kernel<192, true>); else go(stiffness_mw_multi_kernel<192, false>); }
    covered |= mine;
  }
  return covered;
}


static unsigned launch_stiffness_all_multi(d4est_hip_plan* plan, const double* u, double* Au) {
  const int tw = plan->tuning[D4EST_HIP_TUNE_STIFFNESS_WAVE];
  if (!(tw < 0 || tw == 11) || plan->tuning[D4EST_HIP_TUNE_STIFFNESS_PREFETCH] > 0) return 0u;
  if (plan->tuning[D4EST_HIP_TUNE_STIFFNESS_BIGP] >= 0 && plan->tuning[D4EST_HIP_TUNE_STIFFNESS_BIGP] != 1) return 0u;
  if (plan->tuning[D4EST_HIP_TUNE_STIFFNESS_EO] == 0) return 0u;
  static const bool split = std::getenv("D4EST_HIP_STIFFNESS_SPLIT_LAUNCH") != nullptr;
  if (split) return 0u;
  WaveEoMulti A;
  size_t lds = 0;
  unsigned mine = 0u;
  int wgs = 0, n_eo = 0, n_mw = 0;
  for (size_t i = 0; i < plan->buckets.size() && i < 32; ++i) {
    const Bucket& bk = plan->buckets[i];
    if (bk.n_elem == 0 || bk.N != bk.NQ || A.n == WaveEoMulti::MAXB) continue;
    if (bk.affine && plan->tuning[D4EST_HIP_TUNE_AFFINE] != 0 && plan->d_metric_affine) continue;
    const int j = A.n;
    if (bk.N >= 2 && bk.N <= 8 && bk.d_EBf && bk.n_elem <= 8192) {
      size_t l = 0;
      int epb = 1;
#define X(N_) if (bk.N == N_) { l = WaveCfg<N_, N_>::LDS_BYTES; epb = WaveCfg<N_, N_>::EPB; }
      X(2) X(3) X(4) X(5) X(6) X(7) X(8)
#undef X
      lds = std::max(lds, 2 * l);
      const int units = (bk.n_elem + epb - 1) / epb;
      wgs += (units + 1) / 2;
      A.EBf[j] = bk.d_EBf; A.EGf[j] = bk.d_EGf; A.EBb[j] = bk.d_EBb; A.EGb[j] = bk.d_EGb;
      ++n_eo;
    } else if (bk.N >= 9 && bk.N <= 11 && bk.d_EDq) {
      lds = std::max(lds, (size_t)2 * bk.N * bk.N * (bk.N | 1) * sizeof(double));
      wgs += bk.n_elem;
      A.EBf[j] = bk.d_EBf; A.EGf[j] = bk.d_EDqT; A.EBb[j] = bk.d_EBb; A.EGb[j] = bk.d_EDq;
      ++n_mw;
    } else {
      continue;
    }
    A.n = j + 1;
    A.wg_end[j] = wgs; A.N[j] = bk.N; A.n_elem[j] = bk.n_elem; A.elem_offset[j] = bk.elem_offset; A.wq[j] = bk.d_w;
    mine |= 1u << i;
  }
  if (n_eo == 0 || n_mw == 0) return 0u;
  std::snprintf(plan->last_kernel, sizeof(plan->last_kernel), "d4est_hip::stiffness_all_multi_kernel (%d + %d buckets)", n_eo, n_mw);
  auto go = [&](auto kern) {
    set_lds_limit(kern, lds);
    hipLaunchKernelGGL(kern, dim3(wgs), dim3(128), lds, plan->stream, u, Au, plan->d_metric, plan->d_ns_list, plan->d_qs_list, A);
  };
  if (plan->stream_mode) go(stiffness_all_multi_kernel<true>); else go(stiffness_all_multi_kernel<false>);
  return mine;
}

void launch_stiffness(d4est_hip_plan* plan, const double* u, double* Au) {
  if (!plan->has_geometry) D4EST_HIP_ABORT("apply_stiffness_matrix: d4est_hip_plan_set_geometry was not called");
  unsigned covered = launch_stiffness_all_multi(plan, u, Au);
  if (covered == 0u) covered = launch_stiffness_multi(plan, u, Au) | launch_stiffness_multi_mw(plan, u, Au);
  size_t bucket_index = 0;
  for (const Bucket& bk : plan->buckets) {
    const size_t this_bucket = bucket_index++;
    if (bk.n_elem == 0) continue;
    if (this_bucket < 32 && ((covered >> this_bucket) & 1u)) continue;
    bool done = false;
    const int tw = plan->tuning[D4EST_HIP_TUNE_STIFFNESS_WAVE], tp = plan->tuning[D4EST_HIP_TUNE_STIFFNESS_PREFETCH];
    const bool affine_ok = bk.affine && plan->tuning[D4EST_HIP_TUNE_AFFINE] != 0;
#define D4EST_AFF_ARGS (affine_ok && plan->d_metric_affine ? plan->d_metric_affine + (size_t)6 * bk.elem_offset : (const double*)nullptr), bk.d_w
    const bool use_wave = (tw < 0) ? (bk.n_elem <= 8192 || affine_ok) : (tw != 0);
    const bool use_pf = (tp < 0) ? !use_wave : (tp != 0);
#define X(N_, NQ_)                                                                                              \
  if (!done && bk.N == N_ && bk.NQ == NQ_) {                                                                    \
    using C = VolCfg<N_, NQ_>;                                                                                  \
    if (C::LDS_BYTES <= 160 * 1024) {                                                                           \
      const int grid = (bk.n_elem + C::EPB - 1) / C::EPB;                                                       \
      constexpr bool kWave = (NQ_ * NQ_ <= 64);                                                                 \
      constexpr bool kEven = true;                                                      \
      const bool use_eo = kEven && bk.d_EBf && plan->tuning[D4EST_HIP_TUNE_STIFFNESS_EO] != 0;                  \
      if (kWave && use_wave) {                                               \
        launch_stiffness_wave<N_, (kWave ? NQ_ : N_)>(plan, bk, use_pf, u, Au);                                 \
      } else if (N_ >= 13 && N_ <= 16 && NQ_ == N_ && (plan->tuning[D4EST_HIP_TUNE_STIFFNESS_BIGP] == 2 || (N_ == 16 && plan->tuning[D4EST_HIP_TUNE_STIFFNESS_BIGP] < 0))) { \
        launch_stiffness_mfma16(plan, bk, u, Au);                                                               \
      } else if (!kWave && plan->tuning[D4EST_HIP_TUNE_STIFFNESS_BIGP] != 0) {                                  \
          \
        using W = WaveCfg<N_, NQ_>;                                                                             \
        std::snprintf(plan->last_kernel, sizeof(plan->last_kernel), "d4est_hip::stiffness_wave_kernel<%d,%d,false,%s%s> (%d threads)", N_, NQ_, use_eo ? "eo" : "plain", (use_eo && affine_ok && plan->d_metric_affine) ? ",affine" : "", W::THREADS); \
        if (use_eo) {                                                                                           \
          if (affine_ok && plan->d_metric_affine) {                                                             \
            set_lds_limit(stiffness_wave_kernel<N_, NQ_, false, kEven, true>, W::LDS_BYTES);                    \
            hipLaunchKernelGGL((stiffness_wave_kernel<N_, NQ_, false, kEven, true>), dim3(bk.n_elem), dim3(W::THREADS), W::LDS_BYTES, \
                               plan->stream, u, Au, plan->d_metric, plan->d_ns_list + bk.elem_offset,           \
                               plan->d_qs_list + bk.elem_offset, bk.n_elem, bk.d_EBb, (kMwCollocated<N_, NQ_, false, true> ? bk.d_EDq : bk.d_EGb), bk.d_EBf, (kMwCollocated<N_, NQ_, false, true> ? bk.d_EDqT : bk.d_EGf), 0, D4EST_AFF_ARGS); \
          } else {                                                                                              \
          auto go_mw = [&](auto kern) {    \
            set_lds_limit(kern, W::LDS_BYTES); \
            hipLaunchKernelGGL(kern, dim3(bk.n_elem), dim3(W::THREADS), W::LDS_BYTES, \
                             plan->stream, u, Au, plan->d_metric, plan->d_ns_list + bk.elem_offset,             \
                             plan->d_qs_list + bk.elem_offset, bk.n_elem, bk.d_EBb, (kMwCollocated<N_, NQ_, false, true> ? bk.d_EDq : bk.d_EGb), bk.d_EBf, (kMwCollocated<N_, NQ_, false, true> ? bk.d_EDqT : bk.d_EGf), (plan->tuning[D4EST_HIP_TUNE_STIFFNESS_STAGGER] < 0 ? 0 : plan->tuning[D4EST_HIP_TUNE_STIFFNESS_STAGGER]), (const double*)nullptr, (const double*)nullptr); \
          }; \
          if (plan->stream_mode) go_mw(stiffness_wave_kernel<N_, NQ_, false, kEven, false, true>); \
          else go_mw(stiffness_wave_kernel<N_, NQ_, false, kEven>); \
          }                                                                                                     \
        } else {                                                                                                \
          set_lds_limit(stiffness_wave_kernel<N_, NQ_, false>, W::LDS_BYTES);                                   \
          hipLaunchKernelGGL((stiffness_wave_kernel<N_, NQ_, false>), dim3(bk.n_elem), dim3(W::THREADS), W::LDS_BYTES, \
                             plan->stream, u, Au, plan->d_metric, plan->d_ns_list + bk.elem_offset,             \
                             plan->d_qs_list + bk.elem_offset, bk.n_elem, bk.d_B, bk.d_G, bk.d_BT, bk.d_GT, 0); \
        }                                                                                                       \
      } else {                                                                                                  \
        constexpr bool kCanPF = (NQ_ <= 8);                                                                     \
        const bool pf = kCanPF && use_pf;                                                                       \
        std::snprintf(plan->last_kernel, sizeof(plan->last_kernel), "d4est_hip::stiffness_kernel<%d,%d,%s,%s>", N_, NQ_, pf ? "true" : "false", use_eo ? "eo" : "plain"); \
        const double* o0 = use_eo ? bk.d_EBb : bk.d_B;                                                          \
        const double* o1 = use_eo ? bk.d_EGb : bk.d_G;                                                          \
        const double* o2 = use_eo ? bk.d_EBf : bk.d_BT;                                                         \
        const double* o3 = use_eo ? bk.d_EGf : bk.d_GT;                                                         \
        auto go = [&](auto kern) {                                                                              \
          set_lds_limit(kern, C::LDS_BYTES);                                                                    \
          hipLaunchKernelGGL(kern, dim3(grid), dim3(C::THREADS), C::LDS_BYTES, plan->stream, u, Au, plan->d_metric, \
                             plan->d_ns_list + bk.elem_offset, plan->d_qs_list + bk.elem_offset, bk.n_elem, o0, o1, o2, o3); \
        };                                                                                                      \
        if (pf && use_eo && plan->stream_mode) go(stiffness_kernel<N_, NQ_, kCanPF, kEven, true>);              \
        else if (pf && use_eo) go(stiffness_kernel<N_, NQ_, kCanPF, kEven>);                                    \
        else if (pf) go(stiffness_kernel<N_, NQ_, kCanPF, false>);                                              \
        else if (use_eo) go(stiffness_kernel<N_, NQ_, false, kEven>);                                           \
        else go(stiffness_kernel<N_, NQ_, false, false>);                                                       \
      }                                                                                                         \
      done = true;                                                                                              \
    }                                                                                                           \
  }
    D4EST_HIP_FAST_PAIRS(X)
#undef X
#define X(N_, NQ_)                                                                                              \
  if (!done && bk.N == N_ && bk.NQ == NQ_ && plan->tuning[D4EST_HIP_TUNE_STIFFNESS_BIGP] != 0) {                \
    using W = WaveCfg<N_, NQ_>;                                                                                 \
    static_assert(W::LDS_BYTES <= 160 * 1024, "two-field kernel does not fit the LDS");                         \
    constexpr bool kEven = true;                                                        \
    const bool use_eo = kEven && bk.d_EBf && plan->tuning[D4EST_HIP_TUNE_STIFFNESS_EO] != 0;                    \
    std::snprintf(plan->last_kernel, sizeof(plan->last_kernel), "d4est_hip::stiffness_wave_kernel<%d,%d,false,%s%s> (%d threads)", N_, NQ_, use_eo ? "eo" : "plain", (use_eo && affine_ok && plan->d_metric_affine) ? ",affine" : "", W::THREADS); \
    if (use_eo) {                                                                                               \
      if (affine_ok && plan->d_metric_affine) {                                                                 \
        set_lds_limit(stiffness_wave_kernel<N_, NQ_, false, kEven, true>, W::LDS_BYTES);                        \
        hipLaunchKernelGGL((stiffness_wave_kernel<N_, NQ_, false, kEven, true>), dim3(bk.n_elem), dim3(W::THREADS), W::LDS_BYTES, \
                           plan->stream, u, Au, plan->d_metric, plan->d_ns_list + bk.elem_offset,               \
                           plan->d_qs_list + bk.elem_offset, bk.n_elem, bk.d_EBb, (kMwCollocated<N_, NQ_, false, true> ? bk.d_EDq : bk.d_EGb), bk.d_EBf, (kMwCollocated<N_, NQ_, false, true> ? bk.d_EDqT : bk.d_EGf), 0, D4EST_AFF_ARGS); \
      } else {                                                                                                  \
      auto go_mw = [&](auto kern) {    \
        set_lds_limit(kern, W::LDS_BYTES); \
        hipLaunchKernelGGL(kern, dim3(bk.n_elem), dim3(W::THREADS), W::LDS_BYTES, \
                         plan->stream, u, Au, plan->d_metric, plan->d_ns_list + bk.elem_offset,                 \
                         plan->d_qs_list + bk.elem_offset, bk.n_elem, bk.d_EBb, (kMwCollocated<N_, NQ_, false, true> ? bk.d_EDq : bk.d_EGb), bk.d_EBf, (kMwCollocated<N_, NQ_, false, true> ? bk.d_EDqT : bk.d_EGf), (plan->tuning[D4EST_HIP_TUNE_STIFFNESS_STAGGER] < 0 ? 0 : plan->tuning[D4EST_HIP_TUNE_STIFFNESS_STAGGER]), (const double*)nullptr, (const double*)nullptr); \
      }; \
      if (plan->stream_mode) go_mw(stiffness_wave_kernel<N_, NQ_, false, kEven, false, true>); \
      else go_mw(stiffness_wave_kernel<N_, NQ_, false, kEven>); \
      }                                                                                                         \
    } else {                                                                                                    \
      set_lds_limit(stiffness_wave_kernel<N_, NQ_, false, false>, W::LDS_BYTES);                                \
      hipLaunchKernelGGL((stiffness_wave_kernel<N_, NQ_, false, false>), dim3(bk.n_elem), dim3(W::THREADS), W::LDS_BYTES, \
                         plan->stream, u, Au, plan->d_metric, plan->d_ns_list + bk.elem_offset,                 \
                         plan->d_qs_list + bk.elem_offset, bk.n_elem, bk.d_B, bk.d_G, bk.d_BT, bk.d_GT, 0);     \
    }                                                                                                           \
    done = true;                                                                                                \
  }
    D4EST_HIP_BIG_PAIRS(X)
#undef X
#undef D4EST_AFF_ARGS
    if (!done) {
      std::snprintf(plan->last_kernel, sizeof(plan->last_kernel), "d4est_hip::generic_volume_kernel (N=%d,NQ=%d)", bk.N, bk.NQ);
      launch_generic(plan, bk, 3, u, Au);
    }
  }
  HIP_CHECK(hipGetLastError());
}

template <int MODE>
static void launch_mass_like_mode(d4est_hip_plan* plan, const double* in, double* out, const double* coeff, int which) {
  unsigned covered = 0u;
  if constexpr (MODE == 0 || MODE == 3) {
    if (which == 0 && plan->tuning[D4EST_HIP_TUNE_STIFFNESS_EO] != 0) {
      WaveEoMulti A;
      size_t lds = 0;
      int wgs = 0;
      for (size_t i = 0; i < plan->buckets.size() && i < 32; ++i) {
        const Bucket& bk = plan->buckets[i];
        if (bk.n_elem == 0 || bk.N != bk.NQ || bk.N < 2 || bk.N > 8 || !bk.d_EBf || A.n == WaveEoMulti::MAXB) continue;
        size_t l = 0;
        int epb = 1;
#define X(N_) if (bk.N == N_) { l = WaveCfg<N_, N_>::LDS_BYTES; epb = WaveCfg<N_, N_>::EPB; }
        X(2) X(3) X(4) X(5) X(6) X(7) X(8)
#undef X
        lds = std::max(lds, l);
        wgs += (bk.n_elem + epb - 1) / epb;
        const int j = A.n++;
        A.wg_end[j] = wgs; A.N[j] = bk.N; A.n_elem[j] = bk.n_elem; A.elem_offset[j] = bk.elem_offset;
        A.EBf[j] = bk.d_EBf; A.EBb[j] = bk.d_EBb; A.wq[j] = bk.d_w;
        covered |= 1u << i;
      }
      if (A.n >= 2)
        hipLaunchKernelGGL((mass_like_multi_kernel<MODE>), dim3(wgs), dim3(64), lds, plan->stream, in, out, plan->d_J, plan->d_ns_list,
                           plan->d_qs_list, coeff, A);
      else
        covered = 0u;
    }
  }
  size_t bucket_index = 0;
// ... 308 lines not shown
```

disco4est_amd/csrc/d4est_hip_wave.h:

```cpp
#pragma once
#include <hip/hip_runtime.h>

namespace d4est_hip {

typedef const double __attribute__((address_space(4))) * sdouble_ptr;
__device__ __forceinline__ sdouble_ptr launder(const double* p) {
  unsigned long long v = reinterpret_cast<unsigned long long>(p);
  asm volatile("" : "+s"(v));
  return (sdouble_ptr)v;
}

template <int NI, int NO>
__device__ __forceinline__ void contract_n(const double* __restrict__ opT, const double* x, double* y) {
#pragma unroll
  for (int o0 = 0; o0 < NO; o0 += 8) {
#pragma unroll
    for (int i = 0; i < NI; ++i) {
      sdouble_ptr row = launder(opT + i * NO + o0);
#pragma unroll
      for (int o = 0; o < 8; ++o) {
        if (o0 + o < NO) y[o0 + o] = (i == 0) ? row[o] * x[0] : fma(row[o], x[i], y[o0 + o]);
      }
    }
  }
}

template <int NI, int NO, bool ACC>
__device__ __forceinline__ void contract_t(const double* __restrict__ op, const double* x, double* y) {
#pragma unroll
  for (int o0 = 0; o0 < NO; o0 += 8) {
#pragma unroll
    for (int i = 0; i < NI; ++i) {
      sdouble_ptr row = launder(op + i * NO + o0);
#pragma unroll
      for (int o = 0; o < 8; ++o) {
        if (o0 + o < NO) y[o0 + o] = (i == 0 && !ACC) ? row[o] * x[0] : fma(row[o], x[i], y[o0 + o]);
      }
    }
  }
}

template <int C>
__device__ __forceinline__ void eo_pre(const double* x, double* xe, double* xo) {
#pragma unroll
  for (int c = 0; c < C / 2; ++c) {
    xe[c] = x[c] + x[C - 1 - c];
    xo[c] = x[c] - x[C - 1 - c];
  }
  if constexpr (C % 2 != 0) {
    xe[C / 2] = x[C / 2];
    xo[C / 2] = x[C / 2];
  }
}
template <int R>
__device__ __forceinline__ void eo_post(const double* ab, double* y) {
  constexpr int SP = (R + 1) / 2;
#pragma unroll
  for (int r = 0; r < R / 2; ++r) {
    y[r] = ab[r] + ab[SP + r];
    y[R - 1 - r] = ab[r] - ab[SP + r];
  }
  if constexpr (R % 2 != 0) y[R / 2] = ab[R / 2];
}

__device__ __forceinline__ void sgpr_touch(double v) { asm volatile("" ::"s"(v)); }
__device__ __forceinline__ void launder2_after(const double* pa, const double* pb, double d0, double d1, sdouble_ptr& ra,
                                               sdouble_ptr& rb) {
  unsigned long long va = reinterpret_cast<unsigned long long>(pa), vb = reinterpret_cast<unsigned long long>(pb);
  asm volatile("" : "+s"(va), "+s"(vb) : "s"(d0), "s"(d1));
  ra = (sdouble_ptr)va;
  rb = (sdouble_ptr)vb;
}

#ifndef D4EST_HIP_EO_IMM_ROWS
#define D4EST_HIP_EO_IMM_ROWS 1
#endif
template <int HC, int R, bool ACCA, bool ACCB>
__device__ __forceinline__ void contract_pair_eo(const double* __restrict__ opA, const double* xfA, const double* xsA, double* yA,
                                                 const double* __restrict__ opB, const double* xfB, const double* xsB, double* yB) {
  constexpr int HR = (R + 1) / 2;
  double ca[R], cb[R], na[R], nb[R];
#if D4EST_HIP_EO_IMM_ROWS
  unsigned long long bA = reinterpret_cast<unsigned long long>(opA), bB = reinterpret_cast<unsigned long long>(opB);
  asm volatile("" : "+s"(bA), "+s"(bB));
  {
    sdouble_ptr ra = (sdouble_ptr)bA, rb = (sdouble_ptr)bB;
#pragma unroll
    for (int o = 0; o < R; ++o) { ca[o] = ra[o]; cb[o] = rb[o]; }
  }
#else
  {
    sdouble_ptr ra = launder(opA), rb = launder(opB);
#pragma unroll
    for (int o = 0; o < R; ++o) { ca[o] = ra[o]; cb[o] = rb[o]; }
  }
#endif
#pragma unroll
  for (int i = 0; i < HC; ++i) {
    if (i + 1 < HC) {
#if D4EST_HIP_EO_IMM_ROWS
      asm volatile("" : "+s"(bA), "+s"(bB) : "s"(ca[0]), "s"(cb[0]));
      sdouble_ptr ra = (sdouble_ptr)bA, rb = (sdouble_ptr)bB;
#pragma unroll
      for (int o = 0; o < R; ++o) { na[o] = ra[(i + 1) * R + o]; nb[o] = rb[(i + 1) * R + o]; }
#else
      sdouble_ptr ra, rb;
      launder2_after(opA + (i + 1) * R, opB + (i + 1) * R, ca[0], cb[0], ra, rb);
#pragma unroll
      for (int o = 0; o < R; ++o) { na[o] = ra[o]; nb[o] = rb[o]; }
#endif
    }
#pragma unroll
    for (int o = 0; o < R; ++o) {
      const double xa = (o < HR) ? xfA[i] : xsA[i], xb = (o < HR) ? xfB[i] : xsB[i];
      yA[o] = (i == 0 && !ACCA) ? ca[o] * xa : fma(ca[o], xa, yA[o]);
      yB[o] = (i == 0 && !ACCB) ? cb[o] * xb : fma(cb[o], xb, yB[o]);
    }
    if (i + 1 < HC) {
#pragma unroll
      for (int o = 0; o < R; ++o) { ca[o] = na[o]; cb[o] = nb[o]; }
    }
    __builtin_amdgcn_sched_barrier(0);
  }
}

template <int HC, int R, bool ACC>
__device__ __forceinline__ void contract_single_eo(const double* __restrict__ op, const double* xf, const double* xs, double* y) {
  constexpr int HR = (R + 1) / 2;
  constexpr int STEPS = (HC + 1) / 2;
  double c0[R], c1[R], n0[R], n1[R];
#if D4EST_HIP_EO_IMM_ROWS
  unsigned long long bs = reinterpret_cast<unsigned long long>(op);
  asm volatile("" : "+s"(bs));
  {
    sdouble_ptr r0 = (sdouble_ptr)bs;
#pragma unroll
    for (int o = 0; o < R; ++o) c0[o] = r0[o];
    if (HC > 1) {
#pragma unroll
      for (int o = 0; o < R; ++o) c1[o] = r0[R + o];
    }
  }
#else
  {
    sdouble_ptr r0 = launder(op);
#pragma unroll
    for (int o = 0; o < R; ++o) c0[o] = r0[o];
    if (HC > 1) {
      sdouble_ptr r1 = launder(op + R);
#pragma unroll
      for (int o = 0; o < R; ++o) c1[o] = r1[o];
    }
  }
#endif
#pragma unroll
  for (int st = 0; st < STEPS; ++st) {
    const int i0 = 2 * st, i1 = 2 * st + 1;
    if (i0 + 2 < HC) {
#if D4EST_HIP_EO_IMM_ROWS
      asm volatile("" : "+s"(bs) : "s"(c0[0]), "s"((i1 < HC) ? c1[0] : c0[0]));
      sdouble_ptr r0 = (sdouble_ptr)bs;
#pragma unroll
      for (int o = 0; o < R; ++o) n0[o] = r0[(i0 + 2) * R + o];
      if (i1 + 2 < HC) {
#pragma unroll
        for (int o = 0; o < R; ++o) n1[o] = r0[(i1 + 2) * R + o];
      }
#else
      sdouble_ptr r0, r1;
      launder2_after(op + (i0 + 2) * R, op + ((i1 + 2 < HC) ? (i1 + 2) : (i0 + 2)) * R, c0[0], (i1 < HC) ? c1[0] : c0[0], r0, r1);
#pragma unroll
      for (int o = 0; o < R; ++o) n0[o] = r0[o];
      if (i1 + 2 < HC) {
#pragma unroll
        for (int o = 0; o < R; ++o) n1[o] = r1[o];
      }
#endif
    }
#pragma unroll
    for (int o = 0; o < R; ++o) {
      const double x0 = (o < HR) ? xf[i0] : xs[i0];
      y[o] = (i0 == 0 && !ACC) ? c0[o] * x0 : fma(c0[o], x0, y[o]);
      if (i1 < HC) {
        const double x1 = (o < HR) ? xf[i1] : xs[i1];
        y[o] = fma(c1[o], x1, y[o]);
      }
    }
#pragma unroll
    for (int o = 0; o < R; ++o) {
      if (i0 + 2 < HC) c0[o] = n0[o];
      if (i1 + 2 < HC) c1[o] = n1[o];
    }
    __builtin_amdgcn_sched_barrier(0);
  }
}

template <int HC, int R, bool ACC>
__device__ __forceinline__ void contract_rows_eo(const double* __restrict__ op, const double* xf, const double* xs, double* y) {
  constexpr int HR = (R + 1) / 2;
  double c0[R], n0[R];
  {
    sdouble_ptr r0 = launder(op);
#pragma unroll
    for (int o = 0; o < R; ++o) c0[o] = r0[o];
  }
#pragma unroll
  for (int i = 0; i < HC; ++i) {
    if (i + 1 < HC) {
      sdouble_ptr r0, r1;
      launder2_after(op + (i + 1) * R, op + (i + 1) * R, c0[0], c0[0], r0, r1);
#pragma unroll
      for (int o = 0; o < R; ++o) n0[o] = r0[o];
    }
#pragma unroll
    for (int o = 0; o < R; ++o) {
      const double x0 = (o < HR) ? xf[i] : xs[i];
      y[o] = (i == 0 && !ACC) ? c0[o] * x0 : fma(c0[o], x0, y[o]);
    }
    if (i + 1 < HC) {
#pragma unroll
      for (int o = 0; o < R; ++o) c0[o] = n0[o];
    }
    __builtin_amdgcn_sched_barrier(0);
  }
}

template <int HC, int R, bool ACC>
__device__ __forceinline__ void contract_rows_eo_imm(const double* __restrict__ op, const double* xf, const double* xs, double* y) {
  constexpr int HR = (R + 1) / 2;
  double c0[R], n0[R];
  unsigned long long base = reinterpret_cast<unsigned long long>(op);
  asm volatile("" : "+s"(base));
  {
    sdouble_ptr r0 = (sdouble_ptr)base;
#pragma unroll
    for (int o = 0; o < R; ++o) c0[o] = r0[o];
  }
#pragma unroll
  for (int i = 0; i < HC; ++i) {
    if (i + 1 < HC) {
      asm volatile("" : "+s"(base) : "s"(c0[0]));
      sdouble_ptr r0 = (sdouble_ptr)base;
#pragma unroll
      for (int o = 0; o < R; ++o) n0[o] = r0[(i + 1) * R + o];
    }
#pragma unroll
    for (int o = 0; o < R; ++o) {
      const double x0 = (o < HR) ? xf[i] : xs[i];
      y[o] = (i == 0 && !ACC) ? c0[o] * x0 : fma(c0[o], x0, y[o]);
    }
    if (i + 1 < HC) {
#pragma unroll
      for (int o = 0; o < R; ++o) c0[o] = n0[o];
    }
    __builtin_amdgcn_sched_barrier(0);
  }
}

struct LdPlain {
  __device__ __forceinline__ double operator()(const double* p) const { return *p; }
};
struct LdStream {
  __device__ __forceinline__ double operator()(const double* p) const { return __builtin_nontemporal_load(p); }
};
#define D4EST_HIP_STREAM_FENCE() asm volatile("; stream mode" ::: "memory")
template <class F>
__device__ __forceinline__ void with_ld(bool nt, F&& f) {
  if (nt) {
    D4EST_HIP_STREAM_FENCE();
    f(LdStream{});
    D4EST_HIP_STREAM_FENCE();
  } else {
    f(LdPlain{});
// ... 273 lines not shown
      }
      eo_post<NQ>(ge, gt);
    }
  }

  if (active) {
    if constexpr (AFF) {
      const double* __restrict__ c = affine + (size_t)6 * ei;
      const double c0 = c[0], c1 = c[1], c2 = c[2], c3 = c[3], c4 = c[4], c5 = c[5];
      const double wab = wq[b] * wq[a];
#pragma unroll
      for (int kq = 0; kq < NQ; ++kq) {
        const double w3 = wq[kq] * wab;
        const double r = w3 * gr[kq], s = w3 * gs[kq], t = w3 * gt[kq];
        gr[kq] = c0 * r + c1 * s + c2 * t;
        gs[kq] = c1 * r + c3 * s + c4 * t;
        gt[kq] = c2 * r + c4 * s + c5 * t;
      }
    } else if constexpr (kPipe) {
      const double* __restrict__ m = metric + (size_t)6 * qs + (a + NQ * b);
#pragma unroll
      for (int kq = ME; kq < MD; ++kq)
#pragma unroll
        for (int c = 0; c < 6; ++c) mw[kq][c] = ld_sel<NT>(&m[c * NQ3 + NQ * NQ * kq]);
      __builtin_amdgcn_sched_barrier(0);
#pragma unroll
      for (int kq = 0; kq < NQ; ++kq) {
        if (kq + MD < NQ) {
#pragma unroll
          for (int c = 0; c < 6; ++c) mw[kq + MD][c] = ld_sel<NT>(&m[c * NQ3 + NQ * NQ * (kq + MD)]);
        }
        __builtin_amdgcn_sched_barrier(0);
        const double r = gr[kq], s = gs[kq], t = gt[kq];
        gr[kq] = mw[kq][0] * r + mw[kq][1] * s + mw[kq][2] * t;
        gs[kq] = mw[kq][1] * r + mw[kq][3] * s + mw[kq][4] * t;
        gt[kq] = mw[kq][2] * r + mw[kq][4] * s + mw[kq][5] * t;
        __builtin_amdgcn_sched_barrier(0);
      }
    } else {
      const double* __restrict__ m = metric + (size_t)6 * qs + (a + NQ * b);
#pragma unroll
      for (int kq = 0; kq < NQ; ++kq) {
        const int q = NQ * NQ * kq;
        const double m0 = m[q], m1 = m[NQ3 + q], m2 = m[2 * NQ3 + q], m3 = m[3 * NQ3 + q], m4 = m[4 * NQ3 + q], m5 = m[5 * NQ3 + q];
        const double r = gr[kq], s = gs[kq], t = gt[kq];
        gr[kq] = m0 * r + m1 * s + m2 * t;
        gs[kq] = m1 * r + m3 * s + m4 * t;
        gt[kq] = m2 * r + m4 * s + m5 * t;
      }
    }
  }

  {
    double cc[N], ar[N], bs[N];
    const bool on6 = active && b < N;
    {
      double ca[N], cb[N];
      if (active) {
        double re[HQ], ro[HQ], se[HQ], so[HQ], te_[HQ], to[HQ];
        eo_pre<NQ>(gr, re, ro);
        eo_pre<NQ>(gs, se, so);
        eo_pre<NQ>(gt, te_, to);
        contract_pair_eo<HQ, N, false, false>(EBb, re, ro, ca, EBb, se, so, cb);
        contract_single_eo<HQ, N, false>(EGb, to, te_, cc);
        if constexpr (MASS) {
          const double* __restrict__ cp = cq + qs + (a + NQ * b);
          double cv[NQ], vm[NQ], me[HQ], mo[HQ];
#pragma unroll
          for (int kq = 0; kq < NQ; ++kq) cv[kq] = cp[NQ * NQ * kq];
#pragma unroll
          for (int kq = 0; kq < NQ; ++kq) vm[kq] = lds_ld(&R1[kq * C::PL + (a + NQ * b)]) * cv[kq];
          eo_pre<NQ>(vm, me, mo);
          contract_single_eo<HQ, N, true>(EBb, me, mo, cc);
        }
      }
      SYNC();
      if (active) {
        double y[N];
        eo_post<N>(ca, y);
#pragma unroll
        for (int k = 0; k < N; ++k) R0[b + PQ * (a + NQ * k)] = y[k];
        eo_post<N>(cb, y);
#pragma unroll
        for (int k = 0; k < N; ++k) R1[b + PQ * (a + NQ * k)] = y[k];
      }
    }
    SYNC();
    if (on6) {
      double x[NQ], y[NQ], xe[HQ], xo[HQ], ye[HQ], yo[HQ];
#pragma unroll
      for (int jq = 0; jq < NQ; ++jq) {
        x[jq] = lds_ld(&R0[jq + PQ * (a + NQ * b)]);
        y[jq] = lds_ld(&R1[jq + PQ * (a + NQ * b)]);
      }
      eo_pre<NQ>(x, xe, xo);
      eo_pre<NQ>(y, ye, yo);
      contract_pair_eo<HQ, N, false, false>(EBb, xe, xo, ar, EGb, yo, ye, bs);
    }
    SYNC();
    if (active) {
      double y[N];
      eo_post<N>(cc, y);
#pragma unroll
      for (int k = 0; k < N; ++k) R0[b + PQ * (a + NQ * k)] = y[k];
    }
    SYNC();
    if (on6) {
      double z[NQ], ze[HQ], zo[HQ];
#pragma unroll
      for (int jq = 0; jq < NQ; ++jq) z[jq] = lds_ld(&R0[jq + PQ * (a + NQ * b)]);
      eo_pre<NQ>(z, ze, zo);
      contract_single_eo<HQ, N, true>(EBb, ze, zo, bs);
    }
    SYNC();
    if (on6) {
      double y[N];
      eo_post<N>(ar, y);
#pragma unroll
      for (int j = 0; j < N; ++j) R0[a + PQ * (j + N * b)] = y[j];
      eo_post<N>(bs, y);
#pragma unroll
      for (int j = 0; j < N; ++j) R1[a + PQ * (j + N * b)] = y[j];
    }
  }
  SYNC();

  {
    double o[N], o2[N];
    const bool on = active && a < N && b < N;
    if (on) {
      double x[NQ], y[NQ], xe[HQ], xo[HQ], ye[HQ], yo[HQ];
#pragma unroll
      for (int iq = 0; iq < NQ; ++iq) {
        x[iq] = lds_ld(&R0[iq + PQ * (a + N * b)]);
        y[iq] = lds_ld(&R1[iq + PQ * (a + N * b)]);
      }
      eo_pre<NQ>(x, xe, xo);
      eo_pre<NQ>(y, ye, yo);
      contract_pair_eo<HQ, N, false, false>(EGb, xo, xe, o, EBb, ye, yo, o2);
    }
    SYNC();
    if (on) {
      double y[N];
#pragma unroll
      for (int i = 0; i < N; ++i) o[i] += o2[i];
      eo_post<N>(o, y);
#pragma unroll
      for (int i = 0; i < N; ++i) R0[i + PN * (a + N * b)] = y[i];
    }
  }
  SYNC();
}

template <int N, int NQ, bool WG_SYNC>
__device__ __forceinline__ void stiffness_wave2_element(double* R0, double* R1, const double* __restrict__ metric, int qs, bool active,
                                                        int a, int b, const double* __restrict__ Bop, const double* __restrict__ Gop,
                                                        const double* __restrict__ BopT, const double* __restrict__ GopT) {
  using C = WaveCfg<N, NQ>;
  constexpr int PN = C::PN, PQ = C::PQ;
  constexpr int NQ3 = NQ * NQ * NQ;
  auto SYNC = [] {
    if constexpr (WG_SYNC) __syncthreads();
    else wave_lds_fence();
  };

  {
    double x[N], br[NQ], gr[NQ];
    const bool on = active && a < N && b < N;
    if (on) {
#pragma unroll
      for (int i = 0; i < N; ++i) x[i] = R0[i + PN * (a + N * b)];
      contract_pair<N, NQ, false, false>(BopT, x, br, GopT, x, gr);
    }
    SYNC();
    if (on) {
#pragma unroll
      for (int iq = 0; iq < NQ; ++iq) {
        R0[a + PN * (iq + NQ * b)] = br[iq];
        R1[a + PN * (iq + NQ * b)] = gr[iq];
      }
    }
  }
  SYNC();

  double gr[NQ], gs[NQ], gt[NQ];
  {
    double x1[N], x2[N], t1[NQ], t2[NQ], t3[NQ];
    const bool on2 = active && b < N;
    if (on2) {
#pragma unroll
      for (int j = 0; j < N; ++j) {
        x1[j] = R0[j + PN * (a + NQ * b)];
        x2[j] = R1[j + PN * (a + NQ * b)];
      }
      contract_pair<N, NQ, false, false>(BopT, x2, t1, GopT, x1, t2);
      contract_single<N, NQ, false>(BopT, x1, t3);
    }
    SYNC();
    if (on2) {
#pragma unroll
      for (int jq = 0; jq < NQ; ++jq) {
        R0[b + PN * (a + NQ * jq)] = t1[jq];
        R1[b + PN * (a + NQ * jq)] = t2[jq];
      }
    }
    SYNC();
    if (active) {
      double y1[N], y2[N];
#pragma unroll
      for (int k = 0; k < N; ++k) {
        y1[k] = R0[k + PN * (a + NQ * b)];
        y2[k] = R1[k + PN * (a + NQ * b)];
      }
      contract_pair<N, NQ, false, false>(BopT, y1, gr, BopT, y2, gs);
    }
    SYNC();
    if (on2) {
#pragma unroll
      for (int jq = 0; jq < NQ; ++jq) R0[b + PN * (a + NQ * jq)] = t3[jq];
    }
    SYNC();
    if (active) {
      double y3[N];
#pragma unroll
      for (int k = 0; k < N; ++k) y3[k] = R0[k + PN * (a + NQ * b)];
      contract_single<N, NQ, false>(GopT, y3, gt);
    }
  }

  if (active) {
    const double* __restrict__ m = metric + (size_t)6 * qs + (a + NQ * b);
#pragma unroll
    for (int kq = 0; kq < NQ; ++kq) {
      const int q = NQ * NQ * kq;
      const double m0 = m[q], m1 = m[NQ3 + q], m2 = m[2 * NQ3 + q], m3 = m[3 * NQ3 + q], m4 = m[4 * NQ3 + q], m5 = m[5 * NQ3 + q];
      const double r = gr[kq], s = gs[kq], t = gt[kq];
      gr[kq] = m0 * r + m1 * s + m2 * t;
      gs[kq] = m1 * r + m3 * s + m4 * t;
      gt[kq] = m2 * r + m4 * s + m5 * t;
    }
  }

  {
    double ca[N], cb[N], cc[N], ar[N], bs[N];
    const bool on6 = active && b < N;
    if (active) {
      contract_pair<NQ, N, false, false>(Bop, gr, ca, Bop, gs, cb);
      contract_single<NQ, N, false>(Gop, gt, cc);
    }
    SYNC();
    if (active) {
#pragma unroll
      for (int k = 0; k < N; ++k) {
        R0[b + PQ * (a + NQ * k)] = ca[k];
        R1[b + PQ * (a + NQ * k)] = cb[k];
      }
    }
    SYNC();
    if (on6) {
      double x[NQ], y[NQ];
#pragma unroll
      for (int jq = 0; jq < NQ; ++jq) {
        x[jq] = R0[jq + PQ * (a + NQ * b)];
        y[jq] = R1[jq + PQ * (a + NQ * b)];
      }
      contract_pair<NQ, N, false, false>(Bop, x, ar, Gop, y, bs);
    }
    SYNC();
    if (active) {
#pragma unroll
      for (int k = 0; k < N; ++k) R0[b + PQ * (a + NQ * k)] = cc[k];
    }
    SYNC();
    if (on6) {
      double z[NQ];
#pragma unroll
      for (int jq = 0; jq < NQ; ++jq) z[jq] = R0[jq + PQ * (a + NQ * b)];
      contract_single<NQ, N, true>(Bop, z, bs);
    }
    SYNC();
    if (on6) {
#pragma unroll
      for (int j = 0; j < N; ++j) {
        R0[a + PQ * (j + N * b)] = ar[j];
        R1[a + PQ * (j + N * b)] = bs[j];
      }
    }
  }
  SYNC();

  {
    double x[NQ], y[NQ], o[N], o2[N];
    const bool on = active && a < N && b < N;
    if (on) {
#pragma unroll
      for (int iq = 0; iq < NQ; ++iq) {
        x[iq] = R0[iq + PQ * (a + N * b)];
        y[iq] = R1[iq + PQ * (a + N * b)];
      }
      contract_pair<NQ, N, false, false>(Gop, x, o, Bop, y, o2);
    }
    SYNC();
    if (on) {
#pragma unroll
      for (int i = 0; i < N; ++i) R0[i + PN * (a + N * b)] = o[i] + o2[i];
    }
// ... 6 lines not shown
```

Measured before the change: 90.59 GDoF/s.

## Add collocated-derivative stiffness path for N==NQ using quadrature-space differentiation

```diff
diff --git a/disco4est_amd/csrc/d4est_hip_direct.hip b/disco4est_amd/csrc/d4est_hip_direct.hip
--- a/disco4est_amd/csrc/d4est_hip_direct.hip
+++ b/disco4est_amd/csrc/d4est_hip_direct.hip
@@ -75,6 +75,11 @@
 #ifndef D4EST_HIP_DIRECT_NT_MASK
 #define D4EST_HIP_DIRECT_NT_MASK 7
 #endif
+#ifndef D4EST_HIP_DIRECT_COLLOCATED
+#define D4EST_HIP_DIRECT_COLLOCATED 1
+#endif
+template <int N, int NQ>
+inline constexpr bool kDirectCollocated = D4EST_HIP_DIRECT_COLLOCATED && kWaveCollocated<N, NQ>;
 #ifndef D4EST_HIP_DIRECT_GEOM_EARLY
 #define D4EST_HIP_DIRECT_GEOM_EARLY 1
 #endif
@@ -436,7 +441,11 @@
     {
       const DirectVol vl = direct_load_vol(direct_kargs());
       const int qs = __builtin_amdgcn_readfirstlane(vl.qs_stride >= 0 ? vl.qs0 + e * vl.qs_stride : vl.qs_list[e]);
-      stiffness_wave_eo_element<N, NQ, (VOL & 3) == 2, false, (VOL & 4) != 0, (VOL & 8) != 0 && (D4EST_HIP_DIRECT_NT_MASK & 2) != 0>(s_U, s_S, vl.metric, qs, e, on_q, a, b, vl.EBf, vl.EGf, vl.EBb,
+      if constexpr (kDirectCollocated<N, NQ>)
+        stiffness_wave_eo_element_cg<N, (VOL & 3) == 2, false, (VOL & 4) != 0, (VOL & 8) != 0 && (D4EST_HIP_DIRECT_NT_MASK & 2) != 0>(s_U, s_S, vl.metric, qs, e, on_q, a, b, vl.EBf, vl.EDq, vl.EBb,
+                                                                              vl.EDqT, vl.affine, vl.wq, vl.cq);
+      else
+        stiffness_wave_eo_element<N, NQ, (VOL & 3) == 2, false, (VOL & 4) != 0, (VOL & 8) != 0 && (D4EST_HIP_DIRECT_NT_MASK & 2) != 0>(s_U, s_S, vl.metric, qs, e, on_q, a, b, vl.EBf, vl.EGf, vl.EBb,
                                                                               vl.EGb, vl.affine, vl.wq, vl.cq);
     }
     if (on_m) {
@@ -663,7 +672,7 @@
     }
     const char* sm = (!aff && vol_term != 2 && (vol.stream & 1)) ? ",stream" : "";
     if (dh->mw) std::snprintf(plan->last_kernel, sizeof(plan->last_kernel), "d4est_hip::operator_mw_kernel<%d,vol%s%s> (stiffness_wave_kernel body + faces)", dh->N, aff ? ",affine" : "", sm);
-    else std::snprintf(plan->last_kernel, sizeof(plan->last_kernel), "d4est_hip::faces_direct_kernel<%d,%d,vol%s%s> (faces + stiffness_wave_eo body)", dh->N, dh->NQ, aff ? ",affine" : "", sm);
+    else std::snprintf(plan->last_kernel, sizeof(plan->last_kernel), "d4est_hip::faces_direct_kernel<%d,%d,vol%s%s%s> (faces + stiffness_wave_eo body)", dh->N, dh->NQ, aff ? ",affine" : "", sm, (D4EST_HIP_DIRECT_COLLOCATED && D4EST_HIP_WAVE_COLLOCATED && dh->N == dh->NQ && bk.d_EDq) ? ",cg" : "");
   }
   if (dh->mw) {
     launch_direct_mw(plan, dh, u, ghost_trace, Au, cf, robin_c, robin_r, vmode, vol, n, chunk);
diff --git a/disco4est_amd/csrc/d4est_hip_internal.h b/disco4est_amd/csrc/d4est_hip_internal.h
--- a/disco4est_amd/csrc/d4est_hip_internal.h
+++ b/disco4est_amd/csrc/d4est_hip_internal.h
@@ -141,6 +141,8 @@
 };
 
 namespace d4est_hip {
+inline bool tune_wave_eo(int tw) { return tw < 0 || tw == 11 || tw == 12; }
+
 struct TreeMapParams;
 struct CellDesc;
 void launch_analytic_geometry(d4est_hip_plan* plan, const TreeMapParams& P, const CellDesc* d_cells, double root_len);
diff --git a/disco4est_amd/csrc/d4est_hip_volume.hip b/disco4est_amd/csrc/d4est_hip_volume.hip
--- a/disco4est_amd/csrc/d4est_hip_volume.hip
+++ b/disco4est_amd/csrc/d4est_hip_volume.hip
@@ -477,7 +477,7 @@
   }
 }
 
-template <int N, int NQ, bool AFF = false>
+template <int N, int NQ, bool AFF = false, bool CG = false>
 __global__ __launch_bounds__(64, 4) void stiffness_wave_eo_kernel(
     const double* __restrict__ u, double* __restrict__ Au, const double* __restrict__ metric,
     const int* __restrict__ ns_list, const int* __restrict__ qs_list, int n_bucket, const double* __restrict__ EBf,
@@ -513,7 +513,8 @@
     load_element_image<N, PL, PN>(R0, u + ns, te);
   }
   __syncthreads();
-  stiffness_wave_eo_element<N, NQ, AFF, true>(R0, R1, metric, qs, ei, active, a, b, EBf, EGf, EBb, EGb, affine, wq);
+  if constexpr (CG) stiffness_wave_eo_element_cg<N, AFF, true>(R0, R1, metric, qs, ei, active, a, b, EBf, EGf, EBb, EGb, affine, wq);
+  else stiffness_wave_eo_element<N, NQ, AFF, true>(R0, R1, metric, qs, ei, active, a, b, EBf, EGf, EBb, EGb, affine, wq);
   if (active) {
     store_element_image<N, PL, PN>(Au + ns, R0, te);
   }
@@ -533,7 +534,7 @@
   const double* wq[MAXB] = {};
 };
 
-template <int N, bool AFF>
+template <int N, bool AFF, bool CG>
 __device__ __forceinline__ void wave_eo_multi_body(double* smem, int wg, const double* __restrict__ u, double* __restrict__ Au,
                                                    const double* __restrict__ metric, const int* __restrict__ ns_list,
                                                    const int* __restrict__ qs_list, int n_bucket, const double* __restrict__ EBf,
@@ -561,13 +562,14 @@
     load_element_image<N, PL, PN>(R0, u + ns, te);
   }
   __syncthreads();
-  stiffness_wave_eo_element<N, N, AFF, true>(R0, R1, metric, qs, ei, active, a, b, EBf, EGf, EBb, EGb, affine, wq);
+  if constexpr (CG) stiffness_wave_eo_element_cg<N, AFF, true>(R0, R1, metric, qs, ei, active, a, b, EBf, EGf, EBb, EGb, affine, wq);
+  else stiffness_wave_eo_element<N, N, AFF, true>(R0, R1, metric, qs, ei, active, a, b, EBf, EGf, EBb, EGb, affine, wq);
   if (active) {
     store_element_image<N, PL, PN>(Au + ns, R0, te);
   }
 }
 
-template <bool AFF>
+template <bool AFF, bool CG>
 __global__ __launch_bounds__(64, 4) void stiffness_wave_eo_multi_kernel(const double* __restrict__ u, double* __restrict__ Au,
                                                                         const double* __restrict__ metric,
                                                                         const int* __restrict__ ns_list_all,
@@ -587,7 +589,7 @@
   const double* aff = AFF ? affine_all + (size_t)6 * off : nullptr;
 #define D4EST_CASE(N_)                                                                                                            \
   case N_:                                                                                                                        \
-    wave_eo_multi_body<N_, AFF>(smem, wg, u, Au, metric, ns_list_all + off, qs_list_all + off, nb, EBf, EGf, EBb, EGb, aff, wq);   \
+    wave_eo_multi_body<N_, AFF, CG>(smem, wg, u, Au, metric, ns_list_all + off, qs_list_all + off, nb, EBf, EGf, EBb, EGb, aff, wq);   \
     break;
   switch (A.N[bi]) {
     D4EST_CASE(2) D4EST_CASE(3) D4EST_CASE(4) D4EST_CASE(5) D4EST_CASE(6) D4EST_CASE(7) D4EST_CASE(8)
@@ -646,7 +648,7 @@
 }
 
 
-template <bool NT>
+template <bool NT, bool CG>
 __global__ __launch_bounds__(128, D4EST_HIP_MW_WAVES) void stiffness_all_multi_kernel(const double* __restrict__ u, double* __restrict__ Au,
                                                                                     const double* __restrict__ metric,
                                                                                     const int* __restrict__ ns_list_all,
@@ -679,7 +681,8 @@
       load_element_image<N_, PL, PN>(R0, u + ns, te);                                                                                  \
     }                                                                                                                                  \
     wave_lds_fence();                                                                                                                  \
-    stiffness_wave_eo_element<N_, N_, false, false>(R0, R1, metric, qs, ei, active, te % N_, te / N_, EBf, EGf, EBb, EGb, nullptr, nullptr); \
+    if constexpr (CG) stiffness_wave_eo_element_cg<N_, false, false>(R0, R1, metric, qs, ei, active, te % N_, te / N_, EBf, EGf, EBb, EGb, nullptr, nullptr); \
+    else stiffness_wave_eo_element<N_, N_, false, false>(R0, R1, metric, qs, ei, active, te % N_, te / N_, EBf, EGf, EBb, EGb, nullptr, nullptr); \
     if (active) store_element_image<N_, PL, PN>(Au + ns, R0, te);                                                                      \
   } break;
 #define D4EST_CASE_MW(N_)                                                                                                              \
@@ -1289,6 +1292,11 @@
                      per_block, coeff);
 }
 
+static bool wave_collocated(const d4est_hip_plan* plan, const Bucket& bk) {
+  return D4EST_HIP_WAVE_COLLOCATED && bk.N == bk.NQ && bk.N * bk.N <= 64 && bk.d_EDq && bk.d_EDqT &&
+         plan->tuning[D4EST_HIP_TUNE_STIFFNESS_WAVE] != 12;
+}
+
 template <int N, int NQ>
 static void launch_stiffness_wave(d4est_hip_plan* plan, const Bucket& bk, bool use_pf, const double* u, double* Au) {
   if constexpr (NQ * NQ <= 64 && NQ >= N) {
@@ -1299,19 +1307,25 @@
     (void)cus_;
     const int stagger = ts < 0 ? 0 : ts;
     const int tw_ = plan->tuning[D4EST_HIP_TUNE_STIFFNESS_WAVE];
-    const bool use_affine = bk.affine && plan->tuning[D4EST_HIP_TUNE_AFFINE] != 0 && bk.d_EBf && (tw_ == 11 || tw_ < 0);
+    const bool use_affine = bk.affine && plan->tuning[D4EST_HIP_TUNE_AFFINE] != 0 && bk.d_EBf && tune_wave_eo(tw_);
+    const bool cg = wave_collocated(plan, bk);
+    const double* EGf = cg ? bk.d_EDq : bk.d_EGf;
+    const double* EGb = cg ? bk.d_EDqT : bk.d_EGb;
+    auto go = [&](auto kern, const double* affine, const double* wq) {
+      hipLaunchKernelGGL(kern, dim3(grid), dim3(64), W::LDS_BYTES, plan->stream, u, Au, plan->d_metric, plan->d_ns_list + bk.elem_offset,
+                         plan->d_qs_list + bk.elem_offset, bk.n_elem, bk.d_EBf, EGf, bk.d_EBb, EGb, bk.ns0, bk.ns_stride, bk.qs0,
+                         bk.qs_stride, affine, wq);
+    };
     if (use_affine) {
-      std::snprintf(plan->last_kernel, sizeof(plan->last_kernel), "d4est_hip::stiffness_wave_eo_kernel<%d,%d,affine>", N, NQ);
-      hipLaunchKernelGGL((stiffness_wave_eo_kernel<N, NQ, true>), dim3(grid), dim3(64), W::LDS_BYTES, plan->stream, u, Au, plan->d_metric,
-                           plan->d_ns_list + bk.elem_offset, plan->d_qs_list + bk.elem_offset, bk.n_elem, bk.d_EBf, bk.d_EGf,
-                           bk.d_EBb, bk.d_EGb, bk.ns0, bk.ns_stride, bk.qs0, bk.qs_stride,
-                           plan->d_metric_affine + (size_t)6 * bk.elem_offset, bk.d_w);
-    } else if ((tw_ == 11 || tw_ < 0) && bk.d_EBf) {
-      std::snprintf(plan->last_kernel, sizeof(plan->last_kernel), "d4est_hip::stiffness_wave_eo_kernel<%d,%d>", N, NQ);
-      hipLaunchKernelGGL((stiffness_wave_eo_kernel<N, NQ>), dim3(grid), dim3(64), W::LDS_BYTES, plan->stream, u, Au, plan->d_metric,
-                           plan->d_ns_list + bk.elem_offset, plan->d_qs_list + bk.elem_offset, bk.n_elem, bk.d_EBf, bk.d_EGf,
-                           bk.d_EBb, bk.d_EGb, bk.ns0, bk.ns_stride, bk.qs0, bk.qs_stride);
-    } else if (tw_ == 3 || tw_ < 0) {
+      std::snprintf(plan->last_kernel, sizeof(plan->last_kernel), "d4est_hip::stiffness_wave_eo_kernel<%d,%d,affine%s>", N, NQ, cg ? ",cg" : "");
+      const double* aff = plan->d_metric_affine + (size_t)6 * bk.elem_offset;
+      if constexpr (kWaveCollocated<N, NQ>) { if (cg) go(stiffness_wave_eo_kernel<N, NQ, true, true>, aff, bk.d_w); }
+      if (!cg) go(stiffness_wave_eo_kernel<N, NQ, true, false>, aff, bk.d_w);
+    } else if (tune_wave_eo(tw_) && bk.d_EBf) {
+      std::snprintf(plan->last_kernel, sizeof(plan->last_kernel), "d4est_hip::stiffness_wave_eo_kernel<%d,%d%s>", N, NQ, cg ? ",cg" : "");
+      if constexpr (kWaveCollocated<N, NQ>) { if (cg) go(stiffness_wave_eo_kernel<N, NQ, false, true>, nullptr, nullptr); }
+      if (!cg) go(stiffness_wave_eo_kernel<N, NQ, false, false>, nullptr, nullptr);
+    } else if (tw_ == 3 || tune_wave_eo(tw_)) {
       std::snprintf(plan->last_kernel, sizeof(plan->last_kernel), "d4est_hip::stiffness_wave2_kernel<%d,%d>", N, NQ);
       hipLaunchKernelGGL((stiffness_wave2_kernel<N, NQ>), dim3(grid), dim3(64), W::LDS_BYTES, plan->stream, u, Au, plan->d_metric,
                          plan->d_ns_list + bk.elem_offset, plan->d_qs_list + bk.elem_offset, bk.n_elem, bk.d_B, bk.d_G, bk.d_BT,
@@ -1357,13 +1371,14 @@
 
 static unsigned launch_stiffness_multi(d4est_hip_plan* plan, const double* u, double* Au) {
   const int tw = plan->tuning[D4EST_HIP_TUNE_STIFFNESS_WAVE];
-  if (!(tw < 0 || tw == 11) || plan->tuning[D4EST_HIP_TUNE_STIFFNESS_PREFETCH] > 0) return 0u;
+  if (!tune_wave_eo(tw) || plan->tuning[D4EST_HIP_TUNE_STIFFNESS_PREFETCH] > 0) return 0u;
   unsigned covered = 0u;
   for (int aff = 0; aff < 2; ++aff) {
     WaveEoMulti A;
     size_t lds = 0;
     unsigned mine = 0u;
     int wgs = 0;
+    bool all_cg = true;
     for (size_t i = 0; i < plan->buckets.size() && i < 32; ++i) {
       const Bucket& bk = plan->buckets[i];
       if (bk.n_elem == 0 || bk.N != bk.NQ || bk.N < 2 || bk.N > 8 || !bk.d_EBf || A.n == WaveEoMulti::MAXB) continue;
@@ -1378,17 +1393,19 @@
       wgs += (bk.n_elem + epb - 1) / epb;
       const int j = A.n++;
       A.wg_end[j] = wgs; A.N[j] = bk.N; A.n_elem[j] = bk.n_elem; A.elem_offset[j] = bk.elem_offset;
-      A.EBf[j] = bk.d_EBf; A.EGf[j] = bk.d_EGf; A.EBb[j] = bk.d_EBb; A.EGb[j] = bk.d_EGb; A.wq[j] = bk.d_w;
+      const bool cg = wave_collocated(plan, bk);
+      all_cg = all_cg && cg;
+      A.EBf[j] = bk.d_EBf; A.EGf[j] = cg ? bk.d_EDq : bk.d_EGf; A.EBb[j] = bk.d_EBb; A.EGb[j] = cg ? bk.d_EDqT : bk.d_EGb; A.wq[j] = bk.d_w;
       mine |= 1u << i;
     }
     if (A.n < 2) continue;
-    std::snprintf(plan->last_kernel, sizeof(plan->last_kernel), "d4est_hip::stiffness_wave_eo_multi_kernel<%s> (%d buckets)", aff ? "affine" : "general", A.n);
-    if (aff)
-      hipLaunchKernelGGL((stiffness_wave_eo_multi_kernel<true>), dim3(wgs), dim3(64), lds, plan->stream, u, Au, plan->d_metric, plan->d_ns_list,
-                         plan->d_qs_list, plan->d_metric_affine, A);
-    else
-      hipLaunchKernelGGL((stiffness_wave_eo_multi_kernel<false>), dim3(wgs), dim3(64), lds, plan->stream, u, Au, plan->d_metric, plan->d_ns_list,
-                         plan->d_qs_list, (const double*)nullptr, A);
+    std::snprintf(plan->last_kernel, sizeof(plan->last_kernel), "d4est_hip::stiffness_wave_eo_multi_kernel<%s%s> (%d buckets)", aff ? "affine" : "general", all_cg ? ",cg" : "", A.n);
+    auto go = [&](auto kern) {
+      hipLaunchKernelGGL(kern, dim3(wgs), dim3(64), lds, plan->stream, u, Au, plan->d_metric, plan->d_ns_list, plan->d_qs_list,
+                         aff ? plan->d_metric_affine : (const double*)nullptr, A);
+    };
+    if (aff) { if (all_cg) go(stiffness_wave_eo_multi_kernel<true, true>); else go(stiffness_wave_eo_multi_kernel<true, false>); }
+    else { if (all_cg) go(stiffness_wave_eo_multi_kernel<false, true>); else go(stiffness_wave_eo_multi_kernel<false, false>); }
     covered |= mine;
   }
   return covered;
@@ -1432,7 +1449,7 @@
 
 static unsigned launch_stiffness_all_multi(d4est_hip_plan* plan, const double* u, double* Au) {
   const int tw = plan->tuning[D4EST_HIP_TUNE_STIFFNESS_WAVE];
-  if (!(tw < 0 || tw == 11) || plan->tuning[D4EST_HIP_TUNE_STIFFNESS_PREFETCH] > 0) return 0u;
+  if (!tune_wave_eo(tw) || plan->tuning[D4EST_HIP_TUNE_STIFFNESS_PREFETCH] > 0) return 0u;
   if (plan->tuning[D4EST_HIP_TUNE_STIFFNESS_BIGP] >= 0 && plan->tuning[D4EST_HIP_TUNE_STIFFNESS_BIGP] != 1) return 0u;
   if (plan->tuning[D4EST_HIP_TUNE_STIFFNESS_EO] == 0) return 0u;
   static const bool split = std::getenv("D4EST_HIP_STIFFNESS_SPLIT_LAUNCH") != nullptr;
@@ -1441,6 +1458,7 @@
   size_t lds = 0;
   unsigned mine = 0u;
   int wgs = 0, n_eo = 0, n_mw = 0;
+  bool all_cg = true;
   for (size_t i = 0; i < plan->buckets.size() && i < 32; ++i) {
     const Bucket& bk = plan->buckets[i];
     if (bk.n_elem == 0 || bk.N != bk.NQ || A.n == WaveEoMulti::MAXB) continue;
@@ -1455,7 +1473,9 @@
       lds = std::max(lds, 2 * l);
       const int units = (bk.n_elem + epb - 1) / epb;
       wgs += (units + 1) / 2;
-      A.EBf[j] = bk.d_EBf; A.EGf[j] = bk.d_EGf; A.EBb[j] = bk.d_EBb; A.EGb[j] = bk.d_EGb;
+      const bool cg = wave_collocated(plan, bk);
+      all_cg = all_cg && cg;
+      A.EBf[j] = bk.d_EBf; A.EGf[j] = cg ? bk.d_EDq : bk.d_EGf; A.EBb[j] = bk.d_EBb; A.EGb[j] = cg ? bk.d_EDqT : bk.d_EGb;
       ++n_eo;
     } else if (bk.N >= 9 && bk.N <= 11 && bk.d_EDq) {
       lds = std::max(lds, (size_t)2 * bk.N * bk.N * (bk.N | 1) * sizeof(double));
@@ -1470,12 +1490,13 @@
     mine |= 1u << i;
   }
   if (n_eo == 0 || n_mw == 0) return 0u;
-  std::snprintf(plan->last_kernel, sizeof(plan->last_kernel), "d4est_hip::stiffness_all_multi_kernel (%d + %d buckets)", n_eo, n_mw);
+  std::snprintf(plan->last_kernel, sizeof(plan->last_kernel), "d4est_hip::stiffness_all_multi_kernel%s (%d + %d buckets)", all_cg ? "<cg>" : "", n_eo, n_mw);
   auto go = [&](auto kern) {
     set_lds_limit(kern, lds);
     hipLaunchKernelGGL(kern, dim3(wgs), dim3(128), lds, plan->stream, u, Au, plan->d_metric, plan->d_ns_list, plan->d_qs_list, A);
   };
-  if (plan->stream_mode) go(stiffness_all_multi_kernel<true>); else go(stiffness_all_multi_kernel<false>);
+  if (all_cg) { if (plan->stream_mode) go(stiffness_all_multi_kernel<true, true>); else go(stiffness_all_multi_kernel<false, true>); }
+  else { if (plan->stream_mode) go(stiffness_all_multi_kernel<true, false>); else go(stiffness_all_multi_kernel<false, false>); }
   return mine;
 }
 
diff --git a/disco4est_amd/csrc/d4est_hip_wave.h b/disco4est_amd/csrc/d4est_hip_wave.h
--- a/disco4est_amd/csrc/d4est_hip_wave.h
+++ b/disco4est_amd/csrc/d4est_hip_wave.h
@@ -119,6 +119,40 @@
     if (i + 1 < HC) {
 #pragma unroll
       for (int o = 0; o < R; ++o) { ca[o] = na[o]; cb[o] = nb[o]; }
+    }
+    __builtin_amdgcn_sched_barrier(0);
+  }
+}
+
+template <int HC, int R>
+__device__ __forceinline__ void contract_dual_eo(const double* __restrict__ op, const double* xfA, const double* xsA, double* yA,
+                                                 const double* xfB, const double* xsB, double* yB) {
+  constexpr int HR = (R + 1) / 2;
+  double c0[R], n0[R];
+  unsigned long long base = reinterpret_cast<unsigned long long>(op);
+  asm volatile("" : "+s"(base));
+  {
+    sdouble_ptr r0 = (sdouble_ptr)base;
+#pragma unroll
+    for (int o = 0; o < R; ++o) c0[o] = r0[o];
+  }
+#pragma unroll
+  for (int i = 0; i < HC; ++i) {
+    if (i + 1 < HC) {
+      asm volatile("" : "+s"(base) : "s"(c0[0]));
+      sdouble_ptr r0 = (sdouble_ptr)base;
+#pragma unroll
+      for (int o = 0; o < R; ++o) n0[o] = r0[(i + 1) * R + o];
+    }
+#pragma unroll
+    for (int o = 0; o < R; ++o) {
+      const double xa = (o < HR) ? xfA[i] : xsA[i], xb = (o < HR) ? xfB[i] : xsB[i];
+      yA[o] = (i == 0) ? c0[o] * xa : fma(c0[o], xa, yA[o]);
+      yB[o] = (i == 0) ? c0[o] * xb : fma(c0[o], xb, yB[o]);
+    }
+    if (i + 1 < HC) {
+#pragma unroll
+      for (int o = 0; o < R; ++o) c0[o] = n0[o];
     }
     __builtin_amdgcn_sched_barrier(0);
   }
@@ -698,6 +732,241 @@
   SYNC();
 }
 
+#ifndef D4EST_HIP_WAVE_COLLOCATED
+#define D4EST_HIP_WAVE_COLLOCATED 1
+#endif
+template <int N, int NQ>
+inline constexpr bool kWaveCollocated = D4EST_HIP_WAVE_COLLOCATED && N == NQ && (N * N <= 64);
+
+template <int N, bool AFF, bool WG_SYNC, bool MASS = false, bool NT = false>
+__device__ __forceinline__ void stiffness_wave_eo_element_cg(double* R0, double* R1, const double* __restrict__ metric, int qs, int ei,
+                                                             bool active, int a, int b, const double* __restrict__ EBf,
+                                                             const double* __restrict__ EDq, const double* __restrict__ EBb,
+                                                             const double* __restrict__ EDqT, const double* __restrict__ affine,
+                                                             const double* __restrict__ wq, const double* __restrict__ cq = nullptr) {
+  using C = WaveCfg<N, N>;
+  constexpr int P = C::PN;
+  constexpr int N3 = N * N * N;
+  constexpr int H = (N + 1) / 2;
+  auto SYNC = [] {
+    if constexpr (WG_SYNC) __syncthreads();
+    else wave_lds_fence();
+  };
+  const int line = P * (a + N * b);
+
+  if (active) {
+    double x[N], xe[H], xo[H], ab[N], y[N];
+#pragma unroll
+    for (int i = 0; i < N; ++i) x[i] = lds_ld(&R0[i + line]);
+    eo_pre<N>(x, xe, xo);
+    contract_single_eo<H, N, false>(EBf, xe, xo, ab);
+    eo_post<N>(ab, y);
+#pragma unroll
+    for (int iq = 0; iq < N; ++iq) R1[a + P * (iq + N * b)] = y[iq];
+  }
+  SYNC();
+  if (active) {
+    double x[N], xe[H], xo[H], ab[N], y[N];
+#pragma unroll
+    for (int j = 0; j < N; ++j) x[j] = lds_ld(&R1[j + line]);
+    eo_pre<N>(x, xe, xo);
+    contract_single_eo<H, N, false>(EBf, xe, xo, ab);
+    eo_post<N>(ab, y);
+#pragma unroll
+    for (int jq = 0; jq < N; ++jq) R0[b + P * (a + N * jq)] = y[jq];
+  }
+  SYNC();
+  double gt[N];
+  double vm[MASS ? N : 1];
+  if (active) {
+    double x[N], xe[H], xo[H], ab[N], w[N];
+#pragma unroll
+    for (int k = 0; k < N; ++k) x[k] = lds_ld(&R0[k + line]);
+    eo_pre<N>(x, xe, xo);
+    contract_single_eo<H, N, false>(EBf, xe, xo, ab);
+    eo_post<N>(ab, w);
+#pragma unroll
+    for (int kq = 0; kq < N; ++kq) R1[a + P * (b + N * kq)] = w[kq];
+    if constexpr (MASS) {
+#pragma unroll
+      for (int kq = 0; kq < N; ++kq) vm[kq] = w[kq];
+    }
+    eo_pre<N>(w, xe, xo);
+    contract_single_eo<H, N, false>(EDq, xo, xe, ab);
+    eo_post<N>(ab, gt);
+  }
+  SYNC();
+  constexpr bool kPipe = !AFF && WG_SYNC && (D4EST_HIP_WAVE_EO_DEPTH > 0);
+  constexpr int MD = (D4EST_HIP_WAVE_EO_DEPTH < N) ? D4EST_HIP_WAVE_EO_DEPTH : N;
+  constexpr int ME = (D4EST_HIP_WAVE_EO_EARLY < MD) ? D4EST_HIP_WAVE_EO_EARLY : MD;
+  double mw[kPipe ? N : 1][6];
+  {
+    double ys[N], yr[N];
+    if (active) {
+      double z[N], x[N], ze[H], zo[H], xe[H], xo[H];
+#pragma unroll
+      for (int j = 0; j < N; ++j) {
+        z[j] = lds_ld(&R1[a + P * (j + N * b)]);
+        x[j] = lds_ld(&R1[j + line]);
+      }
+      if constexpr (kPipe) {
+        const double* __restrict__ m = metric + (size_t)6 * qs + (a + N * b);
+#pragma unroll
+        for (int kq = 0; kq < ME; ++kq)
+#pragma unroll
+          for (int c = 0; c < 6; ++c) mw[kq][c] = ld_sel<NT>(&m[c * N3 + N * N * kq]);
+        __builtin_amdgcn_sched_barrier(0);
+      }
+      eo_pre<N>(z, ze, zo);
+      eo_pre<N>(x, xe, xo);
+      contract_dual_eo<H, N>(EDq, zo, ze, ys, xo, xe, yr);
+      double y[N];
+      eo_post<N>(ys, y);
+#pragma unroll
+      for (int j = 0; j < N; ++j) R0[b + P * (a + N * j)] = y[j];
+    }
+    SYNC();
+    if (active) {
+      double y[N];
+      eo_post<N>(yr, y);
+#pragma unroll
+      for (int j = 0; j < N; ++j) R1[b + P * (j + N * a)] = y[j];
+    }
+  }
+  SYNC();
+
+  if (active) {
+    if constexpr (MASS) {
+      const double* __restrict__ cp = cq + qs + (a + N * b);
+      double cv[N];
+#pragma unroll
+      for (int kq = 0; kq < N; ++kq) cv[kq] = cp[N * N * kq];
+#pragma unroll
+      for (int kq = 0; kq < N; ++kq) vm[kq] *= cv[kq];
+    }
+    if constexpr (AFF) {
+      const double* __restrict__ c = affine + (size_t)6 * ei;
+      const double c0 = c[0], c1 = c[1], c2 = c[2], c3 = c[3], c4 = c[4], c5 = c[5];
+      const double wab = wq[b] * wq[a];
+#pragma unroll
+      for (int kq = 0; kq < N; ++kq) {
+        const double w3 = wq[kq] * wab;
+        const double r = w3 * lds_ld(&R1[kq + line]), s = w3 * lds_ld(&R0[kq + line]), t = w3 * gt[kq];
+        R1[kq + line] = c0 * r + c1 * s + c2 * t;
+        R0[kq + line] = c1 * r + c3 * s + c4 * t;
+        gt[kq] = c2 * r + c4 * s + c5 * t;
+      }
+    } else if constexpr (kPipe) {
+      const double* __restrict__ m = metric + (size_t)6 * qs + (a + N * b);
+#pragma unroll
+      for (int kq = ME; kq < MD; ++kq)
+#pragma unroll
+        for (int c = 0; c < 6; ++c) mw[kq][c] = ld_sel<NT>(&m[c * N3 + N * N * kq]);
+      double rn = lds_ld(&R1[line]), sn = lds_ld(&R0[line]);
+      __builtin_amdgcn_sched_barrier(0);
+#pragma unroll
+      for (int kq = 0; kq < N; ++kq) {
+        if (kq + MD < N) {
+#pragma unroll
+          for (int c = 0; c < 6; ++c) mw[kq + MD][c] = ld_sel<NT>(&m[c * N3 + N * N * (kq + MD)]);
+        }
+        const double r = rn, s = sn, t = gt[kq];
+        if (kq + 1 < N) {
+          rn = lds_ld(&R1[kq + 1 + line]);
+          sn = lds_ld(&R0[kq + 1 + line]);
+        }
+        __builtin_amdgcn_sched_barrier(0);
+        R1[kq + line] = mw[kq][0] * r + mw[kq][1] * s + mw[kq][2] * t;
+        R0[kq + line] = mw[kq][1] * r + mw[kq][3] * s + mw[kq][4] * t;
+        gt[kq] = mw[kq][2] * r + mw[kq][4] * s + mw[kq][5] * t;
+        __builtin_amdgcn_sched_barrier(0);
+      }
+    } else {
+      const double* __restrict__ m = metric + (size_t)6 * qs + (a + N * b);
+#pragma unroll
+      for (int kq = 0; kq < N; ++kq) {
+        const int q = N * N * kq;
+        const double m0 = m[q], m1 = m[N3 + q], m2 = m[2 * N3 + q], m3 = m[3 * N3 + q], m4 = m[4 * N3 + q], m5 = m[5 * N3 + q];
+        const double r = lds_ld(&R1[kq + line]), s = lds_ld(&R0[kq + line]), t = gt[kq];
+        R1[kq + line] = m0 * r + m1 * s + m2 * t;
+        R0[kq + line] = m1 * r + m3 * s + m4 * t;
+        gt[kq] = m2 * r + m4 * s + m5 * t;
+      }
+    }
+  }
+
+  double ft[N];
+  if (active) {
+    double te_[H], to[H], ab[N];
+    eo_pre<N>(gt, te_, to);
+    contract_single_eo<H, N, false>(EDqT, to, te_, ab);
+    eo_post<N>(ab, ft);
+    if constexpr (MASS) {
+#pragma unroll
+      for (int kq = 0; kq < N; ++kq) ft[kq] += vm[kq];
+    }
+  }
+  SYNC();
+  if (active) {
+    double z[N], x[N], ze[H], zo[H], xe[H], xo[H], ys[N], yr[N], y[N];
+#pragma unroll
+    for (int j = 0; j < N; ++j) {
+      z[j] = lds_ld(&R0[b + P * (a + N * j)]);
+      x[j] = lds_ld(&R1[b + P * (j + N * a)]);
+    }
+    eo_pre<N>(z, ze, zo);
+    eo_pre<N>(x, xe, xo);
+    contract_dual_eo<H, N>(EDqT, zo, ze, ys, xo, xe, yr);
+    eo_post<N>(ys, y);
+#pragma unroll
+    for (int j = 0; j < N; ++j) R0[b + P * (a + N * j)] = y[j];
+    eo_post<N>(yr, y);
+#pragma unroll
+    for (int j = 0; j < N; ++j) R1[b + P * (j + N * a)] = y[j];
+  }
+  SYNC();
+  {
+    double c[N];
+    if (active) {
+      double F[N], fe[H], fo[H];
+#pragma unroll
+      for (int kq = 0; kq < N; ++kq) F[kq] = ft[kq] + (lds_ld(&R0[kq + line]) + lds_ld(&R1[kq + line]));
+      eo_pre<N>(F, fe, fo);
+      contract_single_eo<H, N, false>(EBb, fe, fo, c);
+    }
+    SYNC();
+    if (active) {
+      double y[N];
+      eo_post<N>(c, y);
+#pragma unroll
+      for (int k = 0; k < N; ++k) R0[b + P * (a + N * k)] = y[k];
+    }
+  }
+  SYNC();
+  if (active) {
+    double x[N], xe[H], xo[H], ab[N], y[N];
+#pragma unroll
+    for (int jq = 0; jq < N; ++jq) x[jq] = lds_ld(&R0[jq + line]);
+    eo_pre<N>(x, xe, xo);
+    contract_single_eo<H, N, false>(EBb, xe, xo, ab);
+    eo_post<N>(ab, y);
+#pragma unroll
+    for (int j = 0; j < N; ++j) R1[a + P * (j + N * b)] = y[j];
+  }
+  SYNC();
+  if (active) {
+    double x[N], xe[H], xo[H], ab[N], y[N];
+#pragma unroll
+    for (int iq = 0; iq < N; ++iq) x[iq] = lds_ld(&R1[iq + line]);
+    eo_pre<N>(x, xe, xo);
+    contract_single_eo<H, N, false>(EBb, xe, xo, ab);
+    eo_post<N>(ab, y);
+#pragma unroll
+    for (int i = 0; i < N; ++i) R0[i + line] = y[i];
+  }
+  SYNC();
+}
+
 template <int N, int NQ, bool WG_SYNC>
 __device__ __forceinline__ void stiffness_wave2_element(double* R0, double* R1, const double* __restrict__ metric, int qs, bool active,
                                                         int a, int b, const double* __restrict__ Bop, const double* __restrict__ Gop,
```

Result: faster. 96.02 GDoF/s, median of 6 (+6.0%).
